# interactiveaudiolab/emphases

Hardware: AMD Instinct MI355X
Metric: utterances/s (10 s @16 kHz) whole-node (higher is better)
Workload: dtype f32; 1 GPU; 64 synthetic 10 s 16 kHz utterances per GPU, conv config, random word alignments, ragged batch with per-utterance (B=1) semantics (BASELINE.json configs[1]); utterances_per_gpu=64, frames_per_gpu=64000, words_per_gpu=1882, conv_tile=64, launch=hipGraph replay, batches_in_flight=2, parallelism=utterance-sharded x1, exchange=none (one rank)

## Files before the change

### emphases_amd/csrc/conv_stack.hip

```cpp
#include <type_traits>

#include "common.h"

#ifndef STACK_STAMP
#define STACK_STAMP(slot)
#endif

namespace emph {

typedef float f32x4 __attribute__((ext_vector_type(4)));
typedef float f32x2 __attribute__((ext_vector_type(2)));

constexpr int kStackChannels = 80;
constexpr int kStackMTiles = 5;
constexpr int kStackSteps = kStackChannels / 4;
constexpr int kStackChunkSteps = 4;
constexpr int kStackChunks = kStackSteps / kStackChunkSteps;
constexpr int kStackStepFloats = 6 * kStackMTiles * 64;
constexpr int kStackChunkFloats = kStackChunkSteps * kStackStepFloats;
constexpr int kStackWidth = 256;
constexpr int kStackStride = 260;
constexpr int kStackThreads = 768;
constexpr int kStackMaxLayers = 3;
constexpr int kSpanFields = 8;

__host__ __device__ constexpr int stack_lds_floats() {
    return kStackChannels * kStackStride + 2 * kStackChunkFloats +
           kStackMaxLayers * kStackChannels;
}

template <bool WORD_SUMS>
__global__ __launch_bounds__(kStackThreads) void conv1d_stack_kernel(
    const float* __restrict__ x, int64_t ldx, float* __restrict__ y, int64_t ldy,
    const float* __restrict__ packs, const float* __restrict__ biases, int layers,
    int relu_mask, const int32_t* __restrict__ spans, const int32_t* __restrict__ slot_map) {
    extern __shared__ __align__(16) float lds[];
    float* act = lds;
    float* ring = act + kStackChannels * kStackStride;
    float* bias_lds = ring + 2 * kStackChunkFloats;
    const int lane = threadIdx.x & 63;
    const int wave = __builtin_amdgcn_readfirstlane(threadIdx.x >> 6);
    const bool loader = wave >= 8;

    const int4 span_a = reinterpret_cast<const int4*>(spans)[2 * blockIdx.x];
    const int4 span_b = reinterpret_cast<const int4*>(spans)[2 * blockIdx.x + 1];
    const int owned_first = span_a.y;
    const int64_t column = span_a.z;
    const int count = span_a.w;
    const int owned = span_b.x;
    const int c0 = span_b.y;

    constexpr int kPackFloats = kStackSteps * kStackStepFloats;
    const int total_chunks = layers * kStackChunks;
    auto request = [&](int g, int first, int n) {
        const int layer = g / kStackChunks;
        const float* source = packs + static_cast<int64_t>(layer) * kPackFloats +
                              (g - layer * kStackChunks) * kStackChunkFloats;
        float* target = ring + (g & 1) * kStackChunkFloats;
        constexpr int kQuads = kStackChunkFloats / 4;
        const int each = (kQuads / 64 + n - 1) / n;
        for (int k = 0; k < each; ++k) {
            const int from = min(((wave - first) + k * n) * 64, kQuads - 64);
            __builtin_amdgcn_global_load_lds(
                (const __attribute__((address_space(1))) void*)(source + 4 * (from + lane)),
                (__attribute__((address_space(3))) void*)(target + 4 * from), 16, 0, 0);
        }
    };
    STACK_STAMP(0);

    const int last_quad = (count - 1) & ~3;
    auto fetch = [&](int c, int q) {
        const int p = c0 + 4 * q;
#ifdef STACK_NO_ROWS
        return make_float4(float(p), 0.f, 0.f, 0.f);
#endif
        return *reinterpret_cast<const float4*>(
            x + static_cast<int64_t>(c) * ldx + column + min(p, last_quad));
    };
    auto masked = [&](int q, const float4& v) {
        const int p = c0 + 4 * q;
        return make_float4(p < count ? v.x : 0.f, p + 1 < count ? v.y : 0.f,
                           p + 2 < count ? v.z : 0.f, p + 3 < count ? v.w : 0.f);
    };
    auto deposit = [&](int c, int q, const float4& raw) {
        const float4 v = masked(q, raw);
        float* target = act + c * kStackStride + 4 * q;
        target[1] = v.x;
        *reinterpret_cast<f32x2*>(target + 2) = f32x2{v.y, v.z};
        target[4] = v.w;
    };
    constexpr int kEarlyRows = 16;
    if (loader) {
        constexpr int kStage = 16 * 64 / 256;
        static_assert(kStage == 4, "the s_waitcnt below count these loads");
        f32x4 rows[kStackChunks - 1][kStage];
        float side[kStackChunks - 1];
        const int mine = threadIdx.x - 512;
        const int q = mine & 63;
        const int p = c0 + 4 * q;
        const float* source = x + static_cast<int64_t>(mine >> 6) * ldx + column + min(p, last_quad);
        const uint32_t target = static_cast<uint32_t>(reinterpret_cast<uintptr_t>(
            (__attribute__((address_space(3))) float*)(act + (mine >> 6) * kStackStride + 4 * q)));
        const int side_kind = mine < 64 ? (mine & 3) : 3;
        const int side_p = side_kind == 0 ? c0 - 1 : c0 + kStackWidth + side_kind - 1;
        const bool side_real = side_kind < 3 && side_p >= 0 && side_p < count;
        const float* side_source = x + static_cast<int64_t>((mine >> 2) & 15) * ldx + column +
                                   (side_real ? side_p : 0);
        const uint32_t side_target = static_cast<uint32_t>(reinterpret_cast<uintptr_t>(
            (__attribute__((address_space(3))) float*)(
                act + ((mine >> 2) & 15) * kStackStride +
                (side_kind == 0 ? 0 : kStackWidth + side_kind))));
        auto ask = [&](int chunk) {
#pragma unroll
            for (int round = 0; round < kStage; ++round) {
                const float* address = source + static_cast<int64_t>(16 * chunk + 4 * round) * ldx;
                asm volatile("global_load_dwordx4 %0, %1, off"
                             : "=v"(rows[chunk - 1][round]) : "v"(address) : "memory");
            }
            const float* address = side_source + static_cast<int64_t>(16 * chunk) * ldx;
            asm volatile("global_load_dword %0, %1, off" : "=v"(side[chunk - 1]) : "v"(address) : "memory");
        };
        auto hand_over = [&](int chunk) {
#pragma unroll
            for (int round = 0; round < kStage; ++round) {
                const f32x4 raw = rows[chunk - 1][round];
                const float first = p < count ? raw[0] : 0.f;
                const f32x2 middle = {p + 1 < count ? raw[1] : 0.f, p + 2 < count ? raw[2] : 0.f};
                const float last = p + 3 < count ? raw[3] : 0.f;
                const uint32_t address = target + (16 * chunk + 4 * round) * (kStackStride * 4);
                asm volatile(
                    "ds_write_b32 %0, %1 offset:4\n\t"
                    "ds_write_b64 %0, %2 offset:8\n\t"
                    "ds_write_b32 %0, %3 offset:16"
                    :
                    : "v"(address), "v"(first), "v"(middle), "v"(last)
                    : "memory");
            }
            const float beside = side_real ? side[chunk - 1] : 0.f;
            const uint32_t address = side_target + 16 * chunk * (kStackStride * 4);
            asm volatile("ds_write_b32 %0, %1" : : "v"(address), "v"(beside) : "memory");
        };
#define EMPH_ROWS_HERE(COUNT, STAGE)                                                        \
    asm volatile("s_waitcnt vmcnt(" #COUNT ")"                                              \
                 : "+v"(rows[STAGE][0]), "+v"(rows[STAGE][1]), "+v"(rows[STAGE][2]),        \
                   "+v"(rows[STAGE][3]), "+v"(side[STAGE])::"memory")
        request(1, 8, 4);
        ask(1);
        __builtin_amdgcn_s_barrier();
        ask(2);
        EMPH_ROWS_HERE(5, 0);
        hand_over(1);
        asm volatile("s_waitcnt lgkmcnt(0)" ::: "memory");
        __builtin_amdgcn_s_barrier();
        request(2, 8, 4);
        ask(3);
        EMPH_ROWS_HERE(13, 1);
        hand_over(2);
        asm volatile("s_waitcnt vmcnt(5) lgkmcnt(0)" ::: "memory");
        __builtin_amdgcn_s_barrier();
        request(3, 8, 4);
        ask(4);
        EMPH_ROWS_HERE(13, 2);
        hand_over(3);
        asm volatile("s_waitcnt vmcnt(5) lgkmcnt(0)" ::: "memory");
        __builtin_amdgcn_s_barrier();
        request(4, 8, 4);
        EMPH_ROWS_HERE(8, 3);
        hand_over(4);
#undef EMPH_ROWS_HERE
        for (int g = 4; g < total_chunks; ++g) {
            asm volatile("s_waitcnt vmcnt(0) lgkmcnt(0)" ::: "memory");
            STACK_STAMP(2 + 8 * (g / kStackChunks) + g % kStackChunks);
            __syncthreads();
            if (g + 1 < total_chunks) request(g + 1, 8, 4);
            if ((g + 1) % kStackChunks == 0 && g + 1 < total_chunks) __syncthreads();
        }
        return;
    }
    request(0, 0, 8);
    {
        static_assert(kStackMaxLayers * kStackChannels <= 512, "one bias per thread");
        const bool has_bias = threadIdx.x < layers * kStackChannels;
        const float bias_value = has_bias ? biases[threadIdx.x] : 0.f;
        constexpr int kEarly = kEarlyRows * 64 / 512;
        float4 early[kEarly];
#pragma unroll
        for (int round = 0; round < kEarly; ++round) {
            const int index = threadIdx.x + 512 * round;
            early[round] = fetch(index >> 6, index & 63);
        }
        float side = 0.f;
        const int side_row = threadIdx.x >> 2, side_kind = threadIdx.x & 3;
        if (side_row < kEarlyRows) {
            const float* row = x + static_cast<int64_t>(side_row) * ldx + column;
            const int p = side_kind == 0 ? c0 - 1 : c0 + kStackWidth + side_kind - 1;
            if (side_kind < 3 && p >= 0 && p < count) side = row[p];
        }
#pragma unroll
        for (int round = 0; round < kEarly; ++round) {
            const int index = threadIdx.x + 512 * round;
            deposit(index >> 6, index & 63, early[round]);
        }
        if (side_row < kEarlyRows)
            act[side_row * kStackStride + (side_kind == 0 ? 0 : kStackWidth + side_kind)] = side;
        if (has_bias) bias_lds[threadIdx.x] = bias_value;
    }
    STACK_STAMP(1);

    const int kk = lane >> 4;
    const int col = lane & 15;
    const int tile = wave & 3;
    const int part = wave >> 2;
    constexpr int split = (kStackMTiles + 1) >> 1;
    const int m_begin = part ? split : 0;
    const float* lane_rows = act + kk * kStackStride + 64 * tile + 4 * col;
    const int p_quad = c0 + 64 * tile + 4 * col;

    auto run = [&](auto count_tag) {
        constexpr int COUNT = decltype(count_tag)::value;
        for (int layer = 0; layer < layers; ++layer) {
            f32x4 acc[6][COUNT];
#pragma unroll
            for (int j = 0; j < 6; ++j)
#pragma unroll
                for (int m = 0; m < COUNT; ++m) acc[j][m] = f32x4{0.f, 0.f, 0.f, 0.f};
            float a[6][COUNT], d[6], v[6];
            auto load_b = [&](int step) {
                const float* source = lane_rows + 4 * step * kStackStride;
                const f32x4 first = *reinterpret_cast<const f32x4*>(source);
                const f32x2 second = *reinterpret_cast<const f32x2*>(source + 4);
                d[0] = first[0], d[1] = first[1], d[2] = first[2], d[3] = first[3];
                d[4] = second[0], d[5] = second[1];
            };
            for (int chunk = 0; chunk < kStackChunks; ++chunk) {
                __syncthreads();
                STACK_STAMP(2 + 8 * layer + chunk);
                if (chunk == 0 || layer == 0) load_b(chunk * kStackChunkSteps);
                const float* weights =
                    ring + ((layer * kStackChunks + chunk) & 1) * kStackChunkFloats +
                    (m_begin << 6) + lane;
#pragma unroll
                for (int ks = 0; ks < kStackChunkSteps; ++ks) {
                    const int step = chunk * kStackChunkSteps + ks;
#pragma unroll
                    for (int j = 0; j < 6; ++j)
#pragma unroll
                        for (int m = 0; m < COUNT; ++m)
#ifdef STACK_FEWER_A_READS
                            a[j][m] = (j & 1) ? a[j - 1][m]
                                              : weights[(ks * 6 * kStackMTiles + j * kStackMTiles + m) << 6];
#else
                            a[j][m] = weights[(ks * 6 * kStackMTiles + j * kStackMTiles + m) << 6];
#endif
#ifdef STACK_NO_TRANSFORM
                    for (int j = 0; j < 6; ++j) v[j] = d[j];
#else
                    const float p = fmaf(-4.f, d[2], d[4]);
                    const float q = fmaf(-4.f, d[1], d[3]);
                    const float c = d[4] - d[2];
                    const float e = 2.f * (d[3] - d[1]);
                    v[0] = fmaf(4.f, d[0], fmaf(-5.f, d[2], d[4]));
                    v[1] = p + q;
                    v[2] = p - q;
                    v[3] = c + e;
                    v[4] = c - e;
                    v[5] = fmaf(4.f, d[1], fmaf(-5.f, d[3], d[5]));
#endif
                    if (step + 1 < kStackSteps) load_b(step + 1);
#pragma unroll
                    for (int j = 0; j < 6; ++j)
#pragma unroll
                        for (int m = 0; m < COUNT; ++m)
                            acc[j][m] = __builtin_amdgcn_mfma_f32_16x16x4f32(
                                a[j][m], v[j], acc[j][m], 0, 0, 0);
                }
            }
            const bool relu = (relu_mask >> layer) & 1;
            const bool last = layer == layers - 1;
            const float* bias_row = bias_lds + layer * kStackChannels;
            STACK_STAMP(2 + 8 * layer + 5);
            if (!last) {
                __syncthreads();
#pragma unroll
                for (int m = 0; m < COUNT; ++m) {
                    const int channel0 = 16 * (m_begin + m) + 4 * kk;
                    const f32x4 add = *reinterpret_cast<const f32x4*>(bias_row + channel0);
#pragma unroll
                    for (int r = 0; r < 4; ++r) {
                        const float m1 = acc[1][m][r], m2 = acc[2][m][r];
                        const float m3 = acc[3][m][r], m4 = acc[4][m][r];
                        const float s12 = m1 + m2, d12 = m1 - m2, s34 = m3 + m4, d34 = m3 - m4;
                        float o0 = acc[0][m][r] + s12 + s34 + add[r];
                        float o1 = fmaf(2.f, d34, d12) + add[r];
                        float o2 = fmaf(4.f, s34, s12) + add[r];
                        float o3 = fmaf(8.f, d34, d12) + acc[5][m][r] + add[r];
                        if (relu) {
                            o0 = o0 < 0.f ? 0.f : o0;
                            o1 = o1 < 0.f ? 0.f : o1;
                            o2 = o2 < 0.f ? 0.f : o2;
                            o3 = o3 < 0.f ? 0.f : o3;
                        }
                        o0 = p_quad < count ? o0 : 0.f;
                        o1 = p_quad + 1 < count ? o1 : 0.f;
                        o2 = p_quad + 2 < count ? o2 : 0.f;
                        o3 = p_quad + 3 < count ? o3 : 0.f;
                        float* target =
                            act + (channel0 + r) * kStackStride + 64 * tile + 4 * col + 1;
                        target[0] = o0;
                        *reinterpret_cast<f32x2*>(target + 1) = f32x2{o1, o2};
                        target[3] = o3;
                    }
                }
                STACK_STAMP(2 + 8 * layer + 6);
                continue;
            }
            const int t = p_quad;
            const int owned_end = owned_first + owned;
            if (WORD_SUMS) {
                int4 slots = {-1, -1, -1, -1};
                if (t < count) slots = *reinterpret_cast<const int4*>(slot_map + column + t);
#pragma unroll
                for (int m = 0; m < COUNT; ++m) {
                    const int channel0 = 16 * (m_begin + m) + 4 * kk;
                    const f32x4 add = *reinterpret_cast<const f32x4*>(bias_row + channel0);
                    f32x4 sum[4];
#pragma unroll
                    for (int r = 0; r < 4; ++r) {
                        const float m1 = acc[1][m][r], m2 = acc[2][m][r];
                        const float m3 = acc[3][m][r], m4 = acc[4][m][r];
                        const float s12 = m1 + m2, d12 = m1 - m2, s34 = m3 + m4, d34 = m3 - m4;
                        float o0 = acc[0][m][r] + s12 + s34 + add[r];
                        float o1 = fmaf(2.f, d34, d12) + add[r];
                        float o2 = fmaf(4.f, s34, s12) + add[r];
                        float o3 = fmaf(8.f, d34, d12) + acc[5][m][r] + add[r];
                        if (relu) {
                            o0 = o0 < 0.f ? 0.f : o0;
                            o1 = o1 < 0.f ? 0.f : o1;
                            o2 = o2 < 0.f ? 0.f : o2;
                            o3 = o3 < 0.f ? 0.f : o3;
                        }
                        o0 = (t >= owned_first && t < owned_end) ? o0 : 0.f;
                        o1 = (t + 1 >= owned_first && t + 1 < owned_end) ? o1 : 0.f;
                        o2 = (t + 2 >= owned_first && t + 2 < owned_end) ? o2 : 0.f;
                        o3 = (t + 3 >= owned_first && t + 3 < owned_end) ? o3 : 0.f;
                        o1 += o0;
                        o2 += o1;
                        o3 += o2;
                        float scan = o3;
                        scan += __builtin_bit_cast(float, __builtin_amdgcn_update_dpp(
                            0, __builtin_bit_cast(int, scan), 0x111, 0xf, 0xf, true));
                        scan += __builtin_bit_cast(float, __builtin_amdgcn_update_dpp(
                            0, __builtin_bit_cast(int, scan), 0x112, 0xf, 0xf, true));
                        scan += __builtin_bit_cast(float, __builtin_amdgcn_update_dpp(
                            0, __builtin_bit_cast(int, scan), 0x114, 0xf, 0xf, true));
                        scan += __builtin_bit_cast(float, __builtin_amdgcn_update_dpp(
                            0, __builtin_bit_cast(int, scan), 0x118, 0xf, 0xf, true));
                        const float before = scan - o3;
                        sum[0][r] = o0 + before;
                        sum[1][r] = o1 + before;
                        sum[2][r] = o2 + before;
                        sum[3][r] = o3 + before;
                    }
#pragma unroll
                    for (int j = 0; j < 4; ++j) {
                        const int slot = j == 0 ? slots.x : j == 1 ? slots.y : j == 2 ? slots.z : slots.w;
                        if (slot >= 0 && t + j >= owned_first && t + j < owned_end)
                            *reinterpret_cast<f32x4*>(y + static_cast<int64_t>(slot) * ldy +
                                                      channel0) = sum[j];
                    }
                }
                continue;
            }
            const bool vector_ok = (ldy & 3) == 0 && (column & 3) == 0 &&
                                   (reinterpret_cast<uintptr_t>(y) & 15) == 0;
#pragma unroll
            for (int m = 0; m < COUNT; ++m) {
                const int channel0 = 16 * (m_begin + m) + 4 * kk;
                const f32x4 add = *reinterpret_cast<const f32x4*>(bias_row + channel0);
#pragma unroll
                for (int r = 0; r < 4; ++r) {
                    const float m1 = acc[1][m][r], m2 = acc[2][m][r];
                    const float m3 = acc[3][m][r], m4 = acc[4][m][r];
                    const float s12 = m1 + m2, d12 = m1 - m2, s34 = m3 + m4, d34 = m3 - m4;
                    float4 out;
                    out.x = acc[0][m][r] + s12 + s34 + add[r];
                    out.y = fmaf(2.f, d34, d12) + add[r];
                    out.z = fmaf(4.f, s34, s12) + add[r];
                    out.w = fmaf(8.f, d34, d12) + acc[5][m][r] + add[r];
                    if (relu) {
                        out.x = out.x < 0.f ? 0.f : out.x;
                        out.y = out.y < 0.f ? 0.f : out.y;
                        out.z = out.z < 0.f ? 0.f : out.z;
                        out.w = out.w < 0.f ? 0.f : out.w;
                    }
                    float* target = y + static_cast<int64_t>(channel0 + r) * ldy + column + t;
                    if (vector_ok && t >= owned_first && t + 3 < owned_end) {
                        *reinterpret_cast<float4*>(target) = out;
                    } else {
                        if (t >= owned_first && t < owned_end) target[0] = out.x;
                        if (t + 1 >= owned_first && t + 1 < owned_end) target[1] = out.y;
                        if (t + 2 >= owned_first && t + 2 < owned_end) target[2] = out.z;
                        if (t + 3 >= owned_first && t + 3 < owned_end) target[3] = out.w;
                    }
                }
            }
            STACK_STAMP(2 + 8 * layer + 6);
        }
    };
    if (part == 0) run(std::integral_constant<int, split>{});
    else run(std::integral_constant<int, kStackMTiles - split>{});
}

}

using namespace emph;

extern "C" {

int32_t emph_conv_stack_max_layers(void) { return kStackMaxLayers; }

int32_t emph_conv_stack_spans(const int64_t* host_counts, const int64_t* host_offsets,
                              int32_t n_segments, int32_t* host_spans) {
    int32_t total = 0;
    for (int32_t segment = 0; segment < n_segments; ++segment) {
        const int64_t count = host_counts[segment];
        if (count <= 0) continue;
        const int64_t quads = (count + 3) / 4;
        int64_t pieces = 1;
        if (quads > 64) {
            pieces = 2;
            while (2 * 63 + (pieces - 2) * 62 < quads) ++pieces;
        }
        const int64_t base = quads / pieces;
        int64_t spare = quads - base * pieces;
        int64_t extra[3] = {0, 0, 0};
        if (pieces > 1) {
            if (spare > 0 && base + 1 <= 63) extra[0] = 1, --spare;
            if (spare > 0 && base + 1 <= 63) extra[1] = 1, --spare;
            extra[2] = spare;
        }
        int64_t done = 0;
        for (int64_t k = 0; k < pieces; ++k) {
            int64_t share = base;
            if (pieces == 1) share = quads;
            else if (k == 0) share += extra[0];
            else if (k == pieces - 1) share += extra[1];
            else if (k <= extra[2]) share += 1;
            if (k == pieces - 1) share = quads - done;
            if (host_spans != nullptr) {
                int32_t* row = host_spans + static_cast<int64_t>(total) * kSpanFields;
                const int64_t first = 4 * done;
                int64_t owned = 4 * share;
                if (first + owned > count) owned = count - first;
                row[0] = segment;
                row[1] = static_cast<int32_t>(first);
                row[2] = static_cast<int32_t>(host_offsets[segment]);
                row[3] = static_cast<int32_t>(count);
                row[4] = static_cast<int32_t>(owned);
                row[5] = static_cast<int32_t>(first > 0 ? first - 4 : 0);
                row[6] = row[7] = 0;
            }
            done += share;
            ++total;
        }
    }
    return total;
}

int emph_conv1d_stack(const float* x, int64_t ldx, float* y, int64_t ldy, const float* packs,
                      const float* biases, int32_t layers, int32_t relu_mask,
                      const int32_t* spans, int32_t n_spans, const int32_t* slot_map,
                      void* stream) {
    if (n_spans == 0) return EMPH_OK;
    EMPH_REQUIRE(x && y && packs && biases && spans, EMPH_EINVAL,
                 "emph_conv1d_stack: null pointer");
    EMPH_REQUIRE(layers >= 1 && layers <= kStackMaxLayers, EMPH_ERANGE,
                 "emph_conv1d_stack: %d layers (1 .. %d)", layers, kStackMaxLayers);
    EMPH_REQUIRE((reinterpret_cast<uintptr_t>(x) & 15) == 0 && (ldx & 3) == 0, EMPH_EINVAL,
                 "emph_conv1d_stack: the input must be 16-byte aligned with ldx a multiple of 4");
    EMPH_REQUIRE(slot_map == nullptr ||
                     ((reinterpret_cast<uintptr_t>(y) & 15) == 0 && (ldy & 3) == 0 &&
                      ldy >= kStackChannels && (reinterpret_cast<uintptr_t>(slot_map) & 15) == 0),
                 EMPH_EINVAL, "emph_conv1d_stack: bad sums buffer or slot map");
    const size_t lds = static_cast<size_t>(stack_lds_floats()) * sizeof(float);
    hipStream_t s = static_cast<hipStream_t>(stream);
    if (slot_map != nullptr) {
        auto kernel = conv1d_stack_kernel<true>;
        static LdsReservation reserved;
        if (int status = reserve_lds(reserved, reinterpret_cast<const void*>(kernel), lds,
                                     "emph_conv1d_stack"))
            return status;
        EMPH_LAUNCH(kernel, dim3(n_spans), dim3(kStackThreads), lds, s, x, ldx, y, ldy, packs,
                    biases, layers, relu_mask, spans, slot_map);
    } else {
        auto kernel = conv1d_stack_kernel<false>;
        static LdsReservation reserved;
        if (int status = reserve_lds(reserved, reinterpret_cast<const void*>(kernel), lds,
                                     "emph_conv1d_stack"))
            return status;
        EMPH_LAUNCH(kernel, dim3(n_spans), dim3(kStackThreads), lds, s, x, ldx, y, ldy, packs,
                    biases, layers, relu_mask, spans, slot_map);
    }
    return check_launch("emph_conv1d_stack");
}

}
```

### emphases_amd/csrc/forward.hip

```cpp
#include "common.h"

using namespace emph;

namespace emph {
__global__ __launch_bounds__(64) void launch_probe_kernel() {}
}

extern "C" {

int emph_launch_probe(void* stream) {
    EMPH_LAUNCH(launch_probe_kernel, dim3(1), dim3(64), 0, static_cast<hipStream_t>(stream));
    return check_launch("emph_launch_probe");
}

int64_t emph_prominence_workspace_floats(int32_t features, int32_t channels,
                                         int64_t ld_frames, int64_t ld_words,
                                         int32_t n_slots) {
    return (static_cast<int64_t>(features) + 2 * channels) * ld_frames +
           static_cast<int64_t>(channels) * (ld_words + n_slots);
}

int emph_prominence_forward(const emph_conv_model* model, const void* audio,
                            int32_t audio_format, const int64_t* seg,
                            const int32_t* frontend_tiles,
                            int32_t n_frontend_tiles, const int32_t* frame_tiles,
                            int32_t n_frame_tiles, int32_t tile_n,
                            const int32_t* word_tiles, int32_t n_word_tiles,
                            const int32_t* bounds, const int32_t* word_segment,
                            int64_t ld_frames, int64_t ld_words, float* workspace,
                            float* logits, float* scores,
                            const emph_word_sum_tables* word_sums,
                            const int32_t* conv_spans, int32_t n_conv_spans, void* stream) {
    EMPH_REQUIRE(model != nullptr, EMPH_EINVAL, "emph_prominence_forward: model is null");
    const emph_conv_model& m = *model;
    EMPH_REQUIRE(audio && seg && workspace, EMPH_EINVAL,
                 "emph_prominence_forward: null pointer");
    EMPH_REQUIRE(m.features == kMels, EMPH_ERANGE,
                 "emph_prominence_forward: %d feature rows (the fused path takes the 80 mel "
                 "rows only)", m.features);
    EMPH_REQUIRE(m.encoder_layers >= 0 && m.encoder_layers <= 16, EMPH_ERANGE,
                 "emph_prominence_forward: %d encoder layers", m.encoder_layers);
    const bool quad = m.conv_variant == 1;
    EMPH_REQUIRE(m.conv_variant == 0 || quad, EMPH_EINVAL,
                 "emph_prominence_forward: conv_variant %d", m.conv_variant);
    EMPH_REQUIRE(!quad || tile_n == 64, EMPH_ERANGE,
                 "emph_prominence_forward: F(4,3) takes 64-position tiles, not %d", tile_n);
    const int64_t lds_square = quad ? emph_conv_winograd4_lds_bytes(m.channels, m.channels)
                                    : emph_conv_winograd_lds_bytes(m.channels, m.channels);
    const int64_t lds_input = quad ? emph_conv_winograd4_lds_bytes(m.channels, m.features)
                                   : emph_conv_winograd_lds_bytes(m.channels, m.features);
    EMPH_REQUIRE(lds_square <= 160 * 1024 && lds_input <= 160 * 1024, EMPH_ERANGE,
                 "emph_prominence_forward: %d channels do not fit the Winograd kernel's LDS",
                 m.channels);
    const int c = m.channels;
    float* features = workspace;
    float* current = features + static_cast<int64_t>(m.features) * ld_frames;
    float* other = current + static_cast<int64_t>(c) * ld_frames;
    float* words = other + static_cast<int64_t>(c) * ld_frames;
    float* sums = words + static_cast<int64_t>(c) * ld_words;
    const bool fold = word_sums != nullptr && m.encoder_layers > 0;
    EMPH_REQUIRE(!fold || (quad && (m.reduction == EMPH_REDUCE_SUM ||
                                    m.reduction == EMPH_REDUCE_AVERAGE)),
                 EMPH_EINVAL,
                 "emph_prominence_forward: word_sums needs conv_variant 1 and a sum / average "
                 "reduction");

    int status = emph_logmel(audio, audio_format, seg, frontend_tiles, n_frontend_tiles, m.table,
                             m.mel_start, m.mel_count, m.mel_offset, m.mel_values, m.mel_nnz,
                             features, ld_frames, 0, -1, nullptr, nullptr, m.normalize, stream);
    if (status) return status;
    auto conv = [&](const float* in, float* out, const float* pack, const float* bias, int c_in,
                    int activation) {
        return quad ? emph_conv1d_winograd4(in, ld_frames, out, ld_frames, pack, bias, c_in, c,
                                            activation, frame_tiles, n_frame_tiles, stream)
                    : emph_conv1d_winograd(in, ld_frames, out, ld_frames, pack, bias, c_in, c,
                                           activation, frame_tiles, n_frame_tiles, tile_n,
                                           stream);
    };
    const int64_t pack_floats =
        quad ? emph_conv_winograd4_pack_size(c, c) : emph_conv_winograd_pack_size(c, c);
    const bool stack = conv_spans != nullptr && quad && c == 80 && m.features == 80 &&
                       m.encoder_packs == m.input_pack + pack_floats &&
                       m.encoder_biases == m.input_bias + c &&
                       (m.activation == EMPH_ACT_RELU || m.activation == EMPH_ACT_NONE);
    if (stack) {
        const int total = 1 + m.encoder_layers;
        const int most = emph_conv_stack_max_layers();
        const int groups = (total + most - 1) / most;
        float* buffers[2] = {current, other};
        const float* in = features;
        int done = 0;
        for (int group = 0; group < groups; ++group) {
            const int size = (total - done + (groups - group) - 1) / (groups - group);
            int relu = 0;
            for (int l = 0; l < size; ++l)
                if (done + l >= 1 && m.activation == EMPH_ACT_RELU) relu |= 1 << l;
            const bool to_sums = group == groups - 1 && fold;
            float* out = to_sums ? sums : buffers[group & 1];
            status = emph_conv1d_stack(in, ld_frames, out, to_sums ? c : ld_frames,
                                       m.input_pack + done * pack_floats,
                                       m.input_bias + static_cast<int64_t>(done) * c, size, relu,
                                       conv_spans, n_conv_spans,
                                       to_sums ? word_sums->slot_map : nullptr, stream);
            if (status) return status;
            in = out;
            done += size;
        }
        current = const_cast<float*>(in);
        status = fold ? emph_word_sums(sums, c, word_sums->terms, word_sums->first,
                                       word_sums->lengths, words, ld_words, c, ld_words,
                                       m.reduction, stream)
                      : emph_segment_reduce(current, ld_frames, bounds, words, ld_words, c, seg,
                                            word_segment, ld_words, m.reduction, stream);
        if (status) return status;
        return emph_word_decoder(words, ld_words, word_tiles, n_word_tiles, c, m.decoder_packs,
                                 m.decoder_biases, m.decoder_layers, m.decoder_kernel_size,
                                 m.activation, m.out_weight, m.out_bias, m.decoder_kernel_size,
                                 m.post, logits, scores, stream);
    }
    status = conv(features, current, m.input_pack, m.input_bias, m.features, EMPH_ACT_NONE);
    if (status) return status;
    for (int layer = 0; layer < m.encoder_layers; ++layer) {
        if (fold && layer == m.encoder_layers - 1) {
            status = emph_conv1d_winograd4_word_sums(
                current, ld_frames, sums, c, m.encoder_packs + layer * pack_floats,
                m.encoder_biases + static_cast<int64_t>(layer) * c, c, c, m.activation,
                frame_tiles, n_frame_tiles, word_sums->slot_map, stream);
            if (status) return status;
            break;
        }
        status = conv(current, other, m.encoder_packs + layer * pack_floats,
                      m.encoder_biases + static_cast<int64_t>(layer) * c, c, m.activation);
        if (status) return status;
        float* swap = current;
        current = other;
        other = swap;
    }
    status = fold ? emph_word_sums(sums, c, word_sums->terms, word_sums->first,
                                   word_sums->lengths, words, ld_words, c, ld_words,
                                   m.reduction, stream)
                  : emph_segment_reduce(current, ld_frames, bounds, words, ld_words, c, seg,
                                        word_segment, ld_words, m.reduction, stream);
    if (status) return status;
    return emph_word_decoder(words, ld_words, word_tiles, n_word_tiles, c, m.decoder_packs,
                             m.decoder_biases, m.decoder_layers, m.decoder_kernel_size,
                             m.activation, m.out_weight, m.out_bias, m.decoder_kernel_size,
                             m.post, logits, scores, stream);
}

}
```

### emphases_amd/engine.py

```python
import contextlib
import functools
import os
import ctypes
import threading

import numpy as np
import torch

from . import config as cfg
from . import melbasis
from . import runtime
from . import weights as weights_module

FRONTEND_BLOCK = None
PRECISIONS = {'f32': (0, 0, 0), 'bf16x3': (2, 32, 3), 'bf16x3_fast': (2, 32, 2),
              'bf16x6': (0, 3, 3)}
ATTENTION_BLOCK = 64
ATTENTION_GROUP = 256
GROUPED_FROM = ATTENTION_GROUP // 2
FUSED_WORDS = 64
EVERYTHING = 1 << 30
SHORT, LONG = (0, GROUPED_FROM - 1), (GROUPED_FROM, EVERYTHING)
FEW_WORDS, MANY_WORDS = (0, FUSED_WORDS), (FUSED_WORDS + 1, EVERYTHING)
WORD_TILE = 16
WINOGRAD_LDS_BUDGET = 160 * 1024
SPLIT16_COLUMNS = 1 << 22
KERNEL_COLUMNS = 1 << 28
HEAD_DIMS = (32, 40, 64)


TRACKS_NEEDED = (
    'pitch/periodicity features come from the third-party '
    '`penn` tracker; pass its outputs as tracks '
    '[2, ld_frames] (see core.from_alignments_and_audios '
    'pitch_tracker=)')


def check_supported(config):
    channels = config.channels
    if channels > 128:
        raise ValueError(f'channels {channels} > 128: the word reduce and '
                         'the LayerNorm hold at most 128 channels')
    if config.architecture == 'transformer':
        head_dim = channels // config.heads
        if head_dim not in HEAD_DIMS:
            raise ValueError(
                f'head dimension {head_dim} (channels {channels} / heads '
                f'{config.heads}) not in {{32, 40, 64}}')
    elif config.layers > 16:
        raise ValueError(f'{config.layers} convolution layers > 16')
    if config.architecture == 'convolution' or not config.has_decoder:
        if channels < 16 or channels % 16:
            raise ValueError(
                f'channels {channels} not a multiple of 16 in 16..128 (the '
                'fused word stage of this configuration)')
        if config.decoder_kernel_size not in (1, 3, 5):
            raise ValueError(
                f'decoder kernel size {config.decoder_kernel_size} not in '
                '{1, 3, 5} (the fused word stage of this configuration)')
        layers = config.layers if config.has_decoder else 0
        if runtime.library().emph_word_decoder_block(
                layers, config.decoder_kernel_size,
                config.decoder_kernel_size) < 16:
            raise ValueError(
                f'{layers} decoder layers of kernel size '
                f'{config.decoder_kernel_size}: the receptive field is too '
                "wide for the fused word stage's 64-word window")


def a_weighting():
    frequencies = np.fft.rfftfreq(n=1024, d=1.0 / 8000)
    f_sq = frequencies ** 2.0
    const = np.array([12194.217, 20.598997, 107.65265, 737.86223]) ** 2.0
    with np.errstate(divide='ignore'):
        weights = 2.0 + 20.0 * (
            np.log10(const[0]) + 2 * np.log10(f_sq)
            - np.log10(f_sq + const[0]) - np.log10(f_sq + const[1])
            - 0.5 * np.log10(f_sq + const[2])
            - 0.5 * np.log10(f_sq + const[3]))
    return (np.maximum(-80.0, weights) - cfg.REF_DB).astype(np.float32)


class _Conv:

    def __init__(self, weight, bias, device, winograd=False):
        weight = np.asarray(weight, dtype=np.float32)
        if weight.ndim == 2:
            weight = weight[:, :, None]
        self.c_out, self.c_in, self.kernel_size = weight.shape
        self.weight = weight
        self.pack = torch.from_numpy(runtime.conv_pack(weight)).to(device)
        self.winograd = None
        if winograd and self.kernel_size == 3 and \
                runtime.conv_winograd_lds_bytes(self.c_out, self.c_in) <= \
                WINOGRAD_LDS_BUDGET:
            self.winograd = torch.from_numpy(
                runtime.conv_winograd_pack(weight)).to(device)
        self.winograd4 = None
        if winograd and self.kernel_size == 3 and self.c_out <= 96 and \
                self.c_in % 4 == 0 and \
                runtime.conv_winograd4_lds_bytes(self.c_out, self.c_in) <= \
                WINOGRAD_LDS_BUDGET:
            self.winograd4 = torch.from_numpy(
                runtime.conv_winograd4_pack(weight)).to(device)
        self.bias = None if bias is None else torch.from_numpy(
            np.ascontiguousarray(bias, dtype=np.float32)).to(device)


class Engine:

    def __init__(self, config=cfg.DEFAULT, state=None, device=None,
                 conv_tile=None, winograd=True, precision='f32'):
        if precision not in PRECISIONS:
            raise ValueError(
                f'precision {precision!r} is not one of {sorted(PRECISIONS)}')
        check_supported(config)
        self.config = config
        self.precision = precision
        self.split_pieces, self.attention_pieces, self.linear_pieces = \
            PRECISIONS[precision]
        self.winograd = winograd
        self.device = runtime.require_gpu(device)
        self.lib = runtime.library()
        global FRONTEND_BLOCK
        FRONTEND_BLOCK = int(self.lib.emph_frontend_block())
        self.conv_tile = conv_tile
        self.timers = None
        self._workspace = {}
        self._staging = {}
        self.lock = threading.RLock()
        self.split_tile = int(os.environ.get('EMPHASES_SPLIT_TILE', 16))
        if self.split_tile not in (16, 32):
            raise ValueError('EMPHASES_SPLIT_TILE must be 16 or 32')
        self.max_columns = SPLIT16_COLUMNS if (
            config.architecture == 'transformer' and self.linear_pieces and
            self.split_tile == 16) else KERNEL_COLUMNS
        state = weights_module.load(state, config)
        self.state = state
        dev = self.device
        to = lambda a: torch.from_numpy(np.ascontiguousarray(a)).to(dev)

        self.table = to(runtime.frontend_table())
        basis = melbasis.default()
        self.mel_start = to(basis.row_start)
        self.mel_count = to(basis.row_count)
        self.mel_offset = to(basis.row_offset)
        self.mel_values = to(basis.values)
        self.mel_nnz = int(basis.values.size)
        self.a_weights = to(a_weighting())

        self.input_layer = _Conv(
            state['input_layer.weight'], state['input_layer.bias'], dev,
            winograd)
        self.frame_encoder = self._stack('frame_encoder')
        self.word_decoder = self._stack('word_decoder') \
            if config.has_decoder else None
        self.output_weight = to(state['output_layer.weight'])
        self.output_bias = to(state['output_layer.bias'])
        self.fused_words = config.architecture == 'convolution' or \
            not config.has_decoder
        self.word_block = WORD_TILE
        if self.fused_words:
            layers = self.word_decoder if config.has_decoder else []
            self.decoder_layers = len(layers)
            self.decoder_packs = torch.from_numpy(np.concatenate([
                runtime.word_decoder_pack(l.weight) for l in layers])).to(dev) \
                if layers else None
            self.decoder_biases = torch.cat([l.bias for l in layers]) \
                if layers else None
            self.word_block = int(self.lib.emph_word_decoder_block(
                self.decoder_layers, config.decoder_kernel_size,
                config.decoder_kernel_size))
            self.decoder_tiles = (runtime.AXIS_DECODER, (
                self.decoder_layers, config.decoder_kernel_size,
                config.decoder_kernel_size))
        if config.architecture == 'transformer':
            self.position = to(weights_module.positional_encoding(
                cfg.MAX_POSITIONS, config.channels))
            self.position_rows = self.position.t().contiguous()
        self.word_transformer = None
        if config.architecture == 'transformer' and config.has_decoder and \
                config.channels in (64, 80) and config.heads == 2 and all(
                    tuple(state[f'word_decoder.model.layers.{i}.{name}.weight']
                          .shape) == (config.channels, config.channels)
                    for i in range(config.layers)
                    for name in ('linear1', 'linear2')):
            self.word_transformer = to(np.concatenate([
                runtime.word_transformer_pack(
                    state, f'word_decoder.model.layers.{i}.', config.channels,
                    config.heads) for i in range(config.layers)]))
        frame_layers = [self.input_layer] + (
            self.frame_encoder if config.architecture == 'convolution' else [])
        self.fuse_qkv = os.environ.get('EMPHASES_FUSE_QKV', '1') != '0'
        self.quad = winograd and config.activation in (None, 'relu') and \
            all(layer.winograd4 is not None for layer in frame_layers)
        self.fold = bool(
            self.quad and config.architecture == 'convolution' and
            config.downsample_location != 'input' and
            config.downsample_method in ('sum', 'average') and
            len(self.frame_encoder) > 0 and config.channels % 4 == 0 and
            os.environ.get('EMPHASES_FOLD_WORD_SUMS', '1') != '0')
        frame_stack = [self.input_layer] + list(self.frame_encoder) \
            if config.architecture == 'convolution' else []
        self.stack = bool(
            self.quad and frame_stack and
            config.downsample_location != 'input' and
            all(layer.c_in == 80 and layer.c_out == 80 and
                layer.kernel_size == 3 and layer.winograd4 is not None
                for layer in frame_stack) and
            os.environ.get('EMPHASES_CONV_STACK', '1') != '0')
        if self.stack:
            self._stack_packs = torch.cat(
                [layer.winograd4 for layer in frame_stack])
            self._stack_biases = torch.cat(
                [layer.bias for layer in frame_stack])
        self.split_conv = bool(self.stack and self.split_pieces == 2)
        self.sum_step = 32 if self.split_conv else 64
        if self.split_conv:
            self._split_packs = to(np.concatenate(
                [runtime.conv_split_pack(layer.weight) for layer in frame_stack]))
        self.model = self._conv_model()

    def lane(self):
        import copy
        other = copy.copy(self)
        other._workspace = {}
        other._staging = {}
        other.timers = None
        other.lock = threading.RLock()
        return other

    def _conv_model(self):
        config = self.config
        layers = [self.input_layer] + (
            self.frame_encoder if config.architecture == 'convolution' else [])
        if config.architecture != 'convolution' or not self.winograd or \
                config.downsample_location == 'input' or \
                config.num_features != cfg.NUM_MELS or \
                any(layer.winograd is None for layer in layers):
            return None
        encoder = self.frame_encoder
        pick = (lambda l: l.winograd4) if self.quad else (lambda l: l.winograd)
        input_pack, input_bias = pick(self.input_layer), self.input_layer.bias
        if self.stack:
            size = input_pack.numel()
            input_pack = self._stack_packs[:size]
            self._encoder_packs = self._stack_packs[size:]
            input_bias = self._stack_biases[:config.channels]
            self._encoder_biases = self._stack_biases[config.channels:]
        else:
            self._encoder_packs = torch.cat([pick(l) for l in encoder]) \
                if encoder else torch.zeros(1, device=self.device)
            self._encoder_biases = torch.cat([l.bias for l in encoder]) \
                if encoder else torch.zeros(1, device=self.device)
        pointer = lambda t: None if t is None else t.data_ptr()
        return runtime.ConvModel(
            channels=config.channels, features=config.num_features,
            encoder_layers=len(encoder), decoder_layers=self.decoder_layers,
            decoder_kernel_size=config.decoder_kernel_size,
            activation=runtime.ACTIVATIONS[config.activation],
            reduction=runtime.REDUCTIONS[config.downsample_method],
            post=runtime.POSTPROCESS[config.loss],
            normalize=int(config.normalize), mel_nnz=self.mel_nnz,
            conv_variant=int(self.quad),
            table=pointer(self.table), mel_start=pointer(self.mel_start),
            mel_count=pointer(self.mel_count),
            mel_offset=pointer(self.mel_offset),
            mel_values=pointer(self.mel_values),
            input_pack=pointer(input_pack),
            input_bias=pointer(input_bias),
            encoder_packs=pointer(self._encoder_packs),
            encoder_biases=pointer(self._encoder_biases),
            decoder_packs=pointer(self.decoder_packs),
            decoder_biases=pointer(self.decoder_biases),
            out_weight=pointer(self.output_weight),
            out_bias=pointer(self.output_bias))

    def _stack(self, prefix):
        config, state, dev = self.config, self.state, self.device
        layers = []
        if config.architecture == 'convolution':
            for i in range(config.layers):
                layers.append(_Conv(
                    state[f'{prefix}.{2 * i}.weight'],
                    state[f'{prefix}.{2 * i}.bias'], dev,
                    self.winograd and prefix == 'frame_encoder'))
            return layers
        channels = config.channels
        to = lambda a: torch.from_numpy(np.ascontiguousarray(a)).to(dev)
        for i in range(config.layers):
            p = f'{prefix}.model.layers.{i}.'
            in_w = state[p + 'self_attn.in_proj_weight']
            in_b = state[p + 'self_attn.in_proj_bias']
            block = None
            square = (channels, channels)
            if channels in (64, 80) and all(
                    tuple(state[p + name].shape) == square for name in (
                        'self_attn.out_proj.weight', 'linear1.weight',
                        'linear2.weight')):
                block = (
                    to(np.concatenate([
                        runtime.linear_chain_pack(
                            state[p + 'self_attn.out_proj.weight'], True),
                        runtime.linear_chain_pack(
                            state[p + 'linear1.weight'], False),
                        runtime.linear_chain_pack(
                            state[p + 'linear2.weight'], False)])),
                    to(np.concatenate([
                        state[p + name].astype(np.float32) for name in (
                            'self_attn.out_proj.bias', 'norm1.weight',
                            'norm1.bias', 'linear1.bias', 'linear2.bias',
                            'norm2.weight', 'norm2.bias')])))
            qkv = None
            if channels in (64, 80):
                qkv = (to(np.concatenate([
                    runtime.linear_chain_pack(
                        in_w[part * channels:(part + 1) * channels], True)
                    for part in range(3)])), to(in_b.astype(np.float32)))
            block_split = qkv_split = None
            if self.linear_pieces and channels == 80 and config.heads == 2 and \
                    block is not None:
                pieces = self.linear_pieces
                pack = functools.partial(
                    runtime.linear_split_pack, pieces=pieces,
                    tile=self.split_tile)
                block_split = (
                    to(np.concatenate([
                        pack(state[p + name])
                        for name in ('self_attn.out_proj.weight',
                                     'linear1.weight', 'linear2.weight')])),
                    block[1])
                qkv_split = (to(np.concatenate([
                    pack(in_w[part * channels:(part + 1) * channels])
                    for part in range(3)])), qkv[1])
            layers.append(dict(
                block=block, qkv=qkv, block_split=block_split,
                qkv_split=qkv_split,
                qk=_Conv(in_w[:2 * channels], in_b[:2 * channels], dev),
                v=_Conv(in_w[2 * channels:], in_b[2 * channels:], dev),
                out=_Conv(state[p + 'self_attn.out_proj.weight'],
                          state[p + 'self_attn.out_proj.bias'], dev),
                linear1=_Conv(state[p + 'linear1.weight'],
                              state[p + 'linear1.bias'], dev),
                linear2=_Conv(state[p + 'linear2.weight'],
                              state[p + 'linear2.bias'], dev),
                norm1=(to(state[p + 'norm1.weight']),
                       to(state[p + 'norm1.bias'])),
                norm2=(to(state[p + 'norm2.weight']),
                       to(state[p + 'norm2.bias']))))
        for i in range(config.layers - 1):
            p = f'{prefix}.model.layers.{i + 1}.'
            block = layers[i]['block']
            layers[i]['block_qkv'] = None
            if block is None or layers[i + 1]['qkv'] is None or \
                    (6 * channels * channels + 10 * channels) * 4 > 160 * 1024:
                continue
            in_w = state[p + 'self_attn.in_proj_weight']
            in_b = state[p + 'self_attn.in_proj_bias']
            layers[i]['block_qkv'] = (
                torch.cat([block[0]] + [to(runtime.linear_chain_pack(
                    in_w[part * channels:(part + 1) * channels], False))
                    for part in range(3)]),
                torch.cat([block[1], to(in_b.astype(np.float32))]))
        if layers:
            layers[-1]['block_qkv'] = None
        return layers


    def frame_tile(self, plan):
        if self.conv_tile is not None and self.conv_tile != 'auto':
            return self.conv_tile
        if self.conv_tile is None and self.quad:
            return 64
        frames = [segment.frames for segment in plan.segments]
        if self.winograd:
            cost = {64: 20.7 if self.quad else 26.7, 32: 23.2, 16: 16.1}
        else:
            cost = {64: 33.5, 32: 31.3, 16: 16.1}
        candidates = (64, 32, 16) if self.quad else (32, 64, 16)
        if self.conv_tile is None and self.winograd:
            candidates = (32, 64)
        best = None
        for tile in candidates:
            tiles = sum(-(-count // tile) for count in frames)
            waves = 4 if tile == 64 else 8
            if tile == 64 and self.quad:
                waves = 4
            groups = -(-tiles // waves)
            trips = -(-groups // 256)
            if best is None or trips * cost[tile] < best[0]:
                best = (trips * cost[tile], tile)
        return best[1]

    def _pinned(self, name, array):
        slots = self._staging.setdefault(name, [[], 0])
        ring, cursor = slots
        if len(ring) < 4:
            ring.append(None)
        index = cursor % len(ring)
        slots[1] = cursor + 1
        tensor = ring[index]
        if tensor is None or tensor.numel() < array.size:
            tensor = torch.empty(
                max(array.size, 1) * 3 // 2, dtype=torch.int32).pin_memory()
            ring[index] = tensor
        view = tensor[:array.size]
        np.copyto(view.numpy(), array)
        return view

    def prepare(self, plan):
        if self.config.downsample_location != 'input':
            tile = self.frame_tile(plan)
            plan.prepared = (tile,) + self._pack(plan, tile, False)
        return plan

    def _pack(self, plan, tile, nested):
        requests = [
            (runtime.AXIS_FRAMES, FRONTEND_BLOCK),
            (runtime.AXIS_FRAMES, tile),
            self.decoder_tiles if self.fused_words
            else (runtime.AXIS_WORDS, self.word_block)]
        if self.config.architecture == 'transformer':
            requests += [(runtime.AXIS_FRAMES, ATTENTION_BLOCK),
                         (runtime.AXIS_FRAMES, ATTENTION_BLOCK) + SHORT,
                         (runtime.AXIS_FRAMES, ATTENTION_GROUP) + LONG,
                         (runtime.AXIS_FRAMES, 32)]
            if self.linear_pieces:
                requests += [(runtime.AXIS_FRAMES, self.split_tile)]
            if not nested:
                requests += [(runtime.AXIS_WORDS, ATTENTION_BLOCK)]
                if self.word_transformer is not None:
                    requests += [
                        (runtime.AXIS_WORDS, ATTENTION_BLOCK) + FEW_WORDS,
                        (runtime.AXIS_WORDS, ATTENTION_BLOCK) + MANY_WORDS,
                        (runtime.AXIS_WORDS, self.word_block) + MANY_WORDS]
        requests = list(dict.fromkeys(requests))
        fold = self.fold and not nested and tile == 64
        stack = self.stack and not nested and tile == 64
        host, offsets = plan.pack_metadata(
            requests, word_sums=fold, spans=stack, sum_step=self.sum_step)
        return host, offsets, fold, stack

    def upload(self, plan, tile=None, nested=False):
        tile = tile or self.frame_tile(plan)
        prepared = getattr(plan, 'prepared', None)
        if prepared is not None and prepared[0] == tile and not nested:
            host, offsets, fold, stack = prepared[1:]
        else:
            host, offsets, fold, stack = self._pack(plan, tile, nested)
        pinned = self._pinned(('meta', nested), host)
        device_buffer = pinned.to(self.device, non_blocking=True)
        views = {'_buffer': device_buffer, '_pinned': pinned, 'tile': tile,
                 'positions': (plan.total_frames, plan.total_words)}
        for name, (start, size) in offsets.items():
            views[name] = (device_buffer[start:start + size], size)
        if fold:
            views['n_slots'] = plan.word_sum_tables(
                plan.stack_restarts(self.sum_step)
                if stack else None)['n_slots']
            views['word_sum_tables'] = runtime.WordSumTables(
                *[views[('word_sums', name)][0].data_ptr() for name in (
                    'slot_map', 'terms', 'first', 'lengths')],
                views['n_slots'])
        if self.config.downsample_location == 'input' and not nested and \
                len(plan):
            pieces = plan.pieces(self.config.downsample_method)
            piece_meta = self.upload(
                pieces.plan, self.frame_tile(pieces.plan), nested=True)
            extra = self._pinned('pieces', np.concatenate([
                pieces.gather.view(np.int32).ravel(),
                pieces.bounds.ravel(), pieces.word_piece,
                pieces.gather[:, 1].astype(np.int32)]))
            extra = extra.to(self.device, non_blocking=True)
            cut = pieces.gather.size * 2
            piece_meta['gather'] = extra[:cut]
            piece_meta['piece_bounds'] = extra[cut:cut + pieces.bounds.size]
            cut += pieces.bounds.size
            piece_meta['word_piece'] = extra[cut:cut + pieces.word_piece.size]
            piece_meta['key_counts'] = extra[cut + pieces.word_piece.size:]
            piece_meta['plan'] = pieces.plan
            piece_meta['_extra'] = extra
            views['pieces'] = piece_meta
        return views


    @contextlib.contextmanager
    def _timed(self, name, flops=0.):
        if self.timers is None:
            yield
            return
        begin = torch.cuda.Event(enable_timing=True)
        end = torch.cuda.Event(enable_timing=True)
        first = self.lib.emph_launch_timer_count()
        begin.record()
        yield
        end.record()
        self.timers.append((name, flops, begin, end, first,
                            self.lib.emph_launch_timer_count()))

    def _buffer(self, name, *shape):
        key = (name, shape)
        tensor = self._workspace.get(key)
        if tensor is None:
            for stale in [k for k in self._workspace if k[0] == name]:
                del self._workspace[stale]
            tensor = torch.empty(shape, dtype=torch.float32, device=self.device)
            self._workspace[key] = tensor
        return tensor

    def pack_audio(self, audios):
        lengths = [int(audio.shape[0]) for audio in audios]
        total = sum(lengths)
        packed = self._buffer('packed_audio', max(total, 1))[:total]
        offset = 0
        for audio, length in zip(audios, lengths):
            packed[offset:offset + length].copy_(audio, non_blocking=True)
            offset += length
        return packed

    def _conv(self, layer, x, ldx, y, ldy, meta, axis, block, activation,
              transpose_out=False, position=False):
        tiles, size = meta[('tiles', axis, block)]
        positions = meta['positions'][axis]
        name = (f'conv1d_{"frames" if axis == runtime.AXIS_FRAMES else "words"}'
                f'_{layer.c_in}x{layer.c_out}_k{layer.kernel_size}')
        flops = 2. * layer.c_in * layer.c_out * layer.kernel_size * positions
        bias = None if layer.bias is None else layer.bias.data_ptr()
        if layer.winograd4 is not None and axis == runtime.AXIS_FRAMES and \
                block == 64 and self.quad and not transpose_out and \
                activation in (None, 'relu'):
            with self._timed(name.replace('conv1d', 'conv1d_winograd4'), flops):
                if position:
                    runtime.check(self.lib.emph_conv1d_winograd4_position(
                        x.data_ptr(), ldx, y.data_ptr(), ldy,
                        layer.winograd4.data_ptr(), bias, layer.c_in,
                        layer.c_out, runtime.ACTIVATIONS[activation],
                        tiles.data_ptr(), size // runtime.TILE_FIELDS,
                        self.position_rows.data_ptr(), cfg.MAX_POSITIONS,
                        runtime.stream()), 'emph_conv1d_winograd4_position')
                    return True
                runtime.check(self.lib.emph_conv1d_winograd4(
                    x.data_ptr(), ldx, y.data_ptr(), ldy,
                    layer.winograd4.data_ptr(), bias, layer.c_in, layer.c_out,
                    runtime.ACTIVATIONS[activation], tiles.data_ptr(),
                    size // runtime.TILE_FIELDS, runtime.stream()),
                    'emph_conv1d_winograd4')
            return False
        if layer.winograd is not None and axis == runtime.AXIS_FRAMES and \
                block in (32, 64) and not transpose_out:
            with self._timed(name.replace('conv1d', 'conv1d_winograd'), flops):
                runtime.check(self.lib.emph_conv1d_winograd(
                    x.data_ptr(), ldx, y.data_ptr(), ldy,
                    layer.winograd.data_ptr(), bias, layer.c_in, layer.c_out,
                    runtime.ACTIVATIONS[activation], tiles.data_ptr(),
                    size // runtime.TILE_FIELDS, block, runtime.stream()),
                    'emph_conv1d_winograd')
            return False
        with self._timed(name, flops):
            runtime.check(self.lib.emph_conv1d(
                x.data_ptr(), ldx, y.data_ptr(), ldy, layer.pack.data_ptr(),
                bias, layer.c_in, layer.c_out, layer.kernel_size,
                runtime.ACTIVATIONS[activation], tiles.data_ptr(),
                size // runtime.TILE_FIELDS, block, int(transpose_out),
                runtime.stream()), 'emph_conv1d')
        return False

    def features(self, audio, plan, meta, tracks=None, config=None, out=None):
        config = config or self.config
        rows = config.num_features
        if out is None:
            out = self._buffer('features', rows, plan.ld_frames)
        elif out.shape[0] < rows or out.stride(0) != plan.ld_frames or \
                out.dtype != torch.float32:
            raise ValueError('features: out must be float32 rows of ld_frames')
        mel_row = 0 if config.mel_feature else -1
        loud_row = rows - 1 if config.loudness_feature else -1
        if config.pitch_feature or config.periodicity_feature:
            if tracks is None or tuple(tracks.shape) != (2, plan.ld_frames):
                raise NotImplementedError(TRACKS_NEEDED)
            first = cfg.NUM_MELS if config.mel_feature else 0
            pitch_row = first if config.pitch_feature else -1
            periodicity_row = first + int(config.pitch_feature) \
                if config.periodicity_feature else -1
            with self._timed('pitch_rows'):
                runtime.check(self.lib.emph_pitch_rows(
                    tracks[0].data_ptr(), tracks[1].data_ptr(),
                    out.data_ptr(), plan.ld_frames, pitch_row,
                    periodicity_row, int(config.normalize),
                    float(np.log2(np.float32(cfg.FMIN))),
                    float(np.log2(np.float32(cfg.FMAX))), runtime.stream()),
                    'emph_pitch_rows')
        tiles, size = meta[('tiles', runtime.AXIS_FRAMES, FRONTEND_BLOCK)]
        count = size // runtime.TILE_FIELDS
        table = meta['table'][0]
        peak = None
        if config.loudness_feature:
            peak = torch.zeros(
                len(plan), dtype=torch.float32, device=self.device)
            with self._timed('frontend_peak'):
                runtime.check(self.lib.emph_frontend_peak(
                    audio.data_ptr(), audio_format(audio), table.data_ptr(),
                    tiles.data_ptr(),
                    count, self.table.data_ptr(), peak.data_ptr(),
                    runtime.stream()), 'emph_frontend_peak')
        if mel_row >= 0 or loud_row >= 0:
            with self._timed('frontend_logmel'):
                runtime.check(self.lib.emph_logmel(
                    audio.data_ptr(), audio_format(audio), table.data_ptr(),
                    tiles.data_ptr(),
                    count, self.table.data_ptr(), self.mel_start.data_ptr(),
                    self.mel_count.data_ptr(), self.mel_offset.data_ptr(),
                    self.mel_values.data_ptr(), self.mel_nnz, out.data_ptr(),
                    plan.ld_frames, mel_row, loud_row,
                    None if peak is None else peak.data_ptr(),
                    self.a_weights.data_ptr(), int(config.normalize),
                    runtime.stream()), 'emph_logmel')
        return out

    def _transformer(self, layers, x, ld, plan, meta, axis, block, tag,
                     key_counts=None, positioned=False, select=()):
        config = self.config
        channels = config.channels
        if block > 32 and ('tiles', axis, 32) + select in meta:
            block = 32
        att_tiles, att_size = meta[('tiles', axis, ATTENTION_BLOCK) + select]
        att_count = att_size // runtime.TILE_FIELDS
        if att_count == 0:
            return x
        counts = plan.frames if axis == runtime.AXIS_FRAMES else plan.words
        if len(counts) and int(counts.max()) > cfg.MAX_POSITIONS:
            raise RuntimeError(
                f'a chunk of {int(counts.max())} positions exceeds the '
                f'{cfg.MAX_POSITIONS}-entry positional encoding; pass a '
                'smaller batch_size')
        if not positioned:
            with self._timed('add_position'):
                runtime.check(self.lib.emph_add_position(
                    x.data_ptr(), ld, self.position.data_ptr(), channels,
                    cfg.MAX_POSITIONS, att_tiles.data_ptr(), att_count,
                    ATTENTION_BLOCK, runtime.stream()), 'emph_add_position')
        qk = self._buffer(tag + '_qk', 2 * channels, ld)
        v = self._buffer(tag + '_v', ld, channels)
        attended = self._buffer(tag + '_attended', channels, ld)
        projected = self._buffer(tag + '_projected', channels, ld)
        attention_flops = 4. * channels * float(
            (counts.astype(np.float64) ** 2).sum())
        launches = [(att_tiles, att_count, ATTENTION_BLOCK)]
        if axis == runtime.AXIS_FRAMES and not select and \
                ('tiles', axis, ATTENTION_GROUP) + LONG in meta:
            launches = []
            for key, size in (((ATTENTION_BLOCK,) + SHORT, ATTENTION_BLOCK),
                              ((ATTENTION_GROUP,) + LONG, ATTENTION_GROUP)):
                tiles, length = meta[('tiles', axis) + key]
                if length:
                    launches.append(
                        (tiles, length // runtime.TILE_FIELDS, size))

        def add_layernorm(norm):
            with self._timed('add_layernorm'):
                runtime.check(self.lib.emph_add_layernorm(
                    x.data_ptr(), projected.data_ptr(), x.data_ptr(), ld,
                    channels, norm[0].data_ptr(), norm[1].data_ptr(),
                    config.layer_norm_eps, 0, ld, runtime.stream()),
                    'emph_add_layernorm')

        split_images = None
        if self.attention_pieces and config.channels // config.heads == 40 and \
                any(tile_n == ATTENTION_GROUP for _, _, tile_n in launches):
            size = int(self.lib.emph_split_kv_bytes(
                ld, len(plan), channels, config.heads,
                self.attention_pieces))
            key = (tag + '_split_kv', (size,))
            split_images = self._workspace.get(key)
            if split_images is None:
                for stale in [k for k in self._workspace if k[0] == key[0]]:
                    del self._workspace[stale]
                split_images = torch.empty(
                    size, dtype=torch.uint8, device=self.device)
                self._workspace[key] = split_images

        projected_images = split_images is not None and \
            all(tile_n == ATTENTION_GROUP for _, _, tile_n in launches)

        def attend(images_written):
            for tiles, count, tile_n in launches:
                counts_pointer = None if key_counts is None else \
                    key_counts.data_ptr()
                if split_images is not None and tile_n == ATTENTION_GROUP:
                    if not images_written:
                        runtime.check(self.lib.emph_split_kv(
                            qk.data_ptr(), v.data_ptr(), ld, channels,
                            config.heads, att_tiles.data_ptr(), att_count,
                            ATTENTION_BLOCK, self.attention_pieces,
                            split_images.data_ptr(), runtime.stream()),
                            'emph_split_kv')
                    runtime.check(self.lib.emph_attention_split(
                        qk.data_ptr(), split_images.data_ptr(),
                        attended.data_ptr(), ld, channels, config.heads,
                        tiles.data_ptr(), count, tile_n, counts_pointer,
                        self.attention_pieces, runtime.stream()),
                        'emph_attention_split')
                    continue
                runtime.check(self.lib.emph_attention(
                    qk.data_ptr(), v.data_ptr(), attended.data_ptr(), ld,
                    channels, config.heads, tiles.data_ptr(), count, tile_n,
                    counts_pointer, runtime.stream()), 'emph_attention')

        split_tiles, wide = None, self.split_tile
        if axis == runtime.AXIS_FRAMES and ('tiles', axis, wide) + select in meta:
            split_tiles = meta[('tiles', axis, wide) + select]

        def position_wise(layer, following):
            tiles, size = split_tiles
            block_packs, vectors = layer['block_split'] if layer else (None, None)
            next_packs, next_bias = following['qkv_split'] if following \
                else (None, None)
            pointer = lambda t: None if t is None else t.data_ptr()
            runtime.check(self.lib.emph_position_wise_split(
                attended.data_ptr() if layer else None, x.data_ptr(), ld,
                channels, config.heads, pointer(block_packs), pointer(vectors),
                pointer(next_packs), pointer(next_bias), self.linear_pieces,
                self.attention_pieces, config.layer_norm_eps,
                runtime.ACTIVATIONS['relu'], tiles.data_ptr(),
                size // runtime.TILE_FIELDS, 16, qk.data_ptr(), v.data_ptr(),
                split_images.data_ptr() if projected_images and following
                else None, runtime.stream()), 'emph_position_wise_split')

        projected_ahead = False
        images_ahead = False
        for index, layer in enumerate(layers):
            split = layer['block_split'] is not None and \
                split_tiles is not None and block <= 32
            images_written = False
            if projected_ahead:
                images_written = images_ahead
            elif split:
                packs, bias = layer['qkv_split']
                tiles, size = split_tiles
                with self._timed(f'qkv_projection_split_{tag}', 6. * channels *
                                 channels * meta['positions'][axis]):
                    if wide == 16:
                        position_wise(None, layer)
                        images_written = projected_images
                    elif projected_images:
                        runtime.check(self.lib.emph_qkv_projection_split_images(
                            x.data_ptr(), ld, qk.data_ptr(),
                            split_images.data_ptr(), channels, config.heads,
                            packs.data_ptr(), self.linear_pieces,
                            self.attention_pieces, bias.data_ptr(),
                            tiles.data_ptr(), size // runtime.TILE_FIELDS, 32,
                            runtime.stream()),
                            'emph_qkv_projection_split_images')
                        images_written = True
                    else:
                        runtime.check(self.lib.emph_qkv_projection_split(
                            x.data_ptr(), ld, qk.data_ptr(), v.data_ptr(),
                            channels, packs.data_ptr(), self.linear_pieces,
                            bias.data_ptr(), tiles.data_ptr(),
                            size // runtime.TILE_FIELDS, 32, runtime.stream()),
                            'emph_qkv_projection_split')
            elif layer['qkv'] is not None and block <= 32:
                packs, bias = layer['qkv']
                tiles, size = meta[('tiles', axis, block) + select]
                with self._timed(f'qkv_projection_{tag}', 6. * channels * channels *
                                 meta['positions'][axis]):
                    runtime.check(self.lib.emph_qkv_projection(
                        x.data_ptr(), ld, qk.data_ptr(), v.data_ptr(),
                        channels, packs.data_ptr(), bias.data_ptr(),
                        tiles.data_ptr(), size // runtime.TILE_FIELDS, block,
                        runtime.stream()), 'emph_qkv_projection')
            else:
                self._conv(layer['qk'], x, ld, qk, ld, meta, axis, block,
                           None)
                self._conv(layer['v'], x, ld, v, channels, meta, axis, block,
                           None, transpose_out=True)
            projected_ahead = False
            with self._timed(f'attention_{tag}', attention_flops):
                attend(images_written)
            following = layers[index + 1] if index + 1 < len(layers) else None
            if split and following is not None and self.fuse_qkv and \
                    following['block_split'] is not None:
                packs, vectors = layer['block_split']
                next_packs, next_bias = following['qkv_split']
                tiles, size = split_tiles
                with self._timed(f'transformer_block_qkv_split_{tag}', 12. *
                                 channels * channels * meta['positions'][axis]):
                    if wide == 16:
                        position_wise(layer, following)
                    else:
                        runtime.check(self.lib.emph_transformer_block_qkv_split(
                            attended.data_ptr(), x.data_ptr(), ld, channels,
                            config.heads, packs.data_ptr(), next_packs.data_ptr(),
                            self.linear_pieces, self.attention_pieces,
                            vectors.data_ptr(), next_bias.data_ptr(),
                            config.layer_norm_eps, runtime.ACTIVATIONS['relu'],
                            tiles.data_ptr(), size // runtime.TILE_FIELDS, 32,
                            qk.data_ptr(), v.data_ptr(),
                            split_images.data_ptr() if projected_images else None,
                            runtime.stream()), 'emph_transformer_block_qkv_split')
                projected_ahead, images_ahead = True, projected_images
                continue
            if split:
                packs, vectors = layer['block_split']
                tiles, size = split_tiles
                with self._timed(f'transformer_block_split_{tag}', 6. * channels *
                                 channels * meta['positions'][axis]):
                    if wide == 16:
                        position_wise(layer, None)
                    else:
                        runtime.check(self.lib.emph_transformer_block_split(
                            attended.data_ptr(), x.data_ptr(), ld, channels,
                            packs.data_ptr(), self.linear_pieces, vectors.data_ptr(),
                            config.layer_norm_eps, runtime.ACTIVATIONS['relu'],
                            tiles.data_ptr(), size // runtime.TILE_FIELDS, 32,
                            runtime.stream()), 'emph_transformer_block_split')
                continue
            if layer['block_qkv'] is not None and block <= 32 and self.fuse_qkv:
                packs, vectors = layer['block_qkv']
                tiles, size = meta[('tiles', axis, block) + select]
                with self._timed(f'transformer_block_qkv_{tag}', 12. * channels *
                                 channels * meta['positions'][axis]):
                    runtime.check(self.lib.emph_transformer_block_qkv(
                        attended.data_ptr(), x.data_ptr(), ld, channels,
                        packs.data_ptr(), vectors.data_ptr(),
                        config.layer_norm_eps, runtime.ACTIVATIONS['relu'],
                        tiles.data_ptr(), size // runtime.TILE_FIELDS, block,
                        qk.data_ptr(), v.data_ptr(), runtime.stream()),
                        'emph_transformer_block_qkv')
                projected_ahead = True
                continue
            if layer['block'] is not None and block <= 32:
                packs, vectors = layer['block']
                tiles, size = meta[('tiles', axis, block) + select]
                with self._timed(f'transformer_block_{tag}', 6. * channels *
                                 channels * meta['positions'][axis]):
                    runtime.check(self.lib.emph_transformer_block(
                        attended.data_ptr(), x.data_ptr(), ld, channels,
                        packs.data_ptr(), vectors.data_ptr(),
                        config.layer_norm_eps, runtime.ACTIVATIONS['relu'],
                        tiles.data_ptr(), size // runtime.TILE_FIELDS, block,
                        runtime.stream()), 'emph_transformer_block')
                continue
            self._conv(layer['out'], attended, ld, projected, ld, meta, axis,
                       block, None)
            add_layernorm(layer['norm1'])
            self._conv(layer['linear1'], x, ld, attended, ld, meta, axis,
                       block, 'relu')
            self._conv(layer['linear2'], attended, ld, projected, ld, meta,
                       axis, block, None)
            add_layernorm(layer['norm2'])
        return x

    def _frame_stack(self, features, ld_f, a, b, out, ld_w, plan, meta,
                     frames=True, words=True):
        config = self.config
        channels = config.channels
        spans, span_size = meta['conv_spans']
        total = 1 + len(self.frame_encoder)
        most = int(self.lib.emph_conv_stack_max_layers())
        groups = -(-total // most)
        fold = 'word_sum_tables' in meta
        view = lambda name: meta[('word_sums', name)][0]
        sums = self._buffer(
            'word_sums', max(meta.get('n_slots', 0), 1), channels)
        pack = self.input_layer.winograd4.numel()
        relu_layers = config.activation == 'relu'
        source, buffers, done = features, (a, b), 0
        if self.split_conv:
            groups = -(-total // 5)
            split_bytes = int(self.lib.emph_conv_split_pack_size())
        for group in range(groups if frames else 0):
            size = -(-(total - done) // (groups - group))
            relu = sum(1 << l for l in range(size)
                       if done + l >= 1 and relu_layers)
            to_sums = fold and group == groups - 1
            target = sums if to_sums else buffers[group & 1]
            flops = 2. * 80 * 80 * 3 * plan.total_frames * size
            if self.split_conv:
                with self._timed('conv1d_split_frames_80x80_k3', flops):
                    runtime.check(self.lib.emph_conv1d_split(
                        source.data_ptr(), ld_f, target.data_ptr(),
                        channels if to_sums else ld_f,
                        self._split_packs[done * split_bytes:].data_ptr(),
                        self._stack_biases[done * channels:].data_ptr(), size,
                        relu, spans.data_ptr(), span_size // 8,
                        view('slot_map').data_ptr() if to_sums else None,
                        runtime.stream()), 'emph_conv1d_split')
                source = target
                done += size
                continue
            with self._timed('conv1d_stack_frames_80x80_k3', flops):
                runtime.check(self.lib.emph_conv1d_stack(
                    source.data_ptr(), ld_f, target.data_ptr(),
                    channels if to_sums else ld_f,
                    self._stack_packs[done * pack:].data_ptr(),
                    self._stack_biases[done * channels:].data_ptr(), size,
                    relu, spans.data_ptr(), span_size // 8,
                    view('slot_map').data_ptr() if to_sums else None,
                    runtime.stream()), 'emph_conv1d_stack')
            source = target
            done += size
        if not words:
            return
        if fold:
            with self._timed('word_sums'):
                runtime.check(self.lib.emph_word_sums(
                    sums.data_ptr(), channels, view('terms').data_ptr(),
                    view('first').data_ptr(), view('lengths').data_ptr(),
                    out.data_ptr(), ld_w, channels, ld_w,
                    runtime.REDUCTIONS[config.downsample_method],
                    runtime.stream()), 'emph_word_sums')
        else:
            with self._timed('segment_reduce'):
                runtime.check(self.lib.emph_segment_reduce(
                    source.data_ptr(), ld_f, meta['bounds'][0].data_ptr(),
                    out.data_ptr(), ld_w, channels,
                    meta['table'][0].data_ptr(),
                    meta['word_segment'][0].data_ptr(), ld_w,
                    runtime.REDUCTIONS[config.downsample_method],
                    runtime.stream()), 'emph_segment_reduce')

    def _word_sums(self, x, ld_f, out, ld_w, plan, meta):
        config = self.config
        layer = self.frame_encoder[-1]
        channels = config.channels
        tiles, size = meta[('tiles', runtime.AXIS_FRAMES, 64)]
        sums = self._buffer('word_sums', max(meta['n_slots'], 1), channels)
        view = lambda name: meta[('word_sums', name)][0]
        flops = 2. * layer.c_in * layer.c_out * 3 * plan.total_frames
        with self._timed(
                f'conv1d_winograd4_frames_{layer.c_in}x{layer.c_out}_k3', flops):
            runtime.check(self.lib.emph_conv1d_winograd4_word_sums(
                x.data_ptr(), ld_f, sums.data_ptr(), channels,
                layer.winograd4.data_ptr(), layer.bias.data_ptr(), layer.c_in,
                layer.c_out, runtime.ACTIVATIONS[config.activation],
                tiles.data_ptr(), size // runtime.TILE_FIELDS,
                view('slot_map').data_ptr(), runtime.stream()),
                'emph_conv1d_winograd4_word_sums')
        with self._timed('word_sums'):
            runtime.check(self.lib.emph_word_sums(
                sums.data_ptr(), channels, view('terms').data_ptr(),
                view('first').data_ptr(), view('lengths').data_ptr(),
                out.data_ptr(), ld_w, channels, ld_w,
                runtime.REDUCTIONS[config.downsample_method],
                runtime.stream()), 'emph_word_sums')

    def _stack_forward(self, layers, x, other, ld, plan, meta, axis, block,
                       tag, key_counts=None, positioned=False):
        config = self.config
        if config.architecture == 'convolution':
            for layer in layers:
                self._conv(layer, x, ld, other, ld, meta, axis, block,
                           config.activation)
                x, other = other, x
            return x
        if axis == runtime.AXIS_WORDS and self.word_transformer is not None \
                and key_counts is None and len(plan.words):
            tiles, size = meta[('tiles', axis, ATTENTION_BLOCK) + FEW_WORDS]
            if size:
                with self._timed('word_transformer'):
                    runtime.check(self.lib.emph_word_transformer(
                        x.data_ptr(), ld, self.position.data_ptr(),
                        cfg.MAX_POSITIONS, config.channels, config.heads,
                        self.word_transformer.data_ptr(), len(layers),
                        config.layer_norm_eps, tiles.data_ptr(),
                        size // runtime.TILE_FIELDS, runtime.stream()),
                        'emph_word_transformer')
            if int(plan.words.max()) > FUSED_WORDS:
                self._transformer(
                    layers, x, ld, plan, meta, axis, block, tag, key_counts,
                    positioned, select=MANY_WORDS)
            return x
        return self._transformer(
            layers, x, ld, plan, meta, axis, block, tag, key_counts, positioned)


    def forward(self, audio, plan, meta=None, stages=None, features=None,
                tracks=None):
        config = self.config
        runs = self.sub_plans(plan)
        if runs is not None:
            if stages is not None:
                raise ValueError(
                    'stages of a plan past the packed-axis limit: pass its '
                    'segments in smaller plans')
            return self._forward_runs(audio, plan, runs, tracks, features)
        meta = meta or self.upload(plan)
        block = meta['tile']
        channels = config.channels
        ld_f, ld_w = plan.ld_frames, plan.ld_words
        frames, words = runtime.AXIS_FRAMES, runtime.AXIS_WORDS
        if self.model is not None and stages is None and features is None \
                and self.timers is None and not self.split_conv and \
                block in ((64,) if self.quad else (32, 64)) and \
                len(plan):
            check_bounds(plan, config.downsample_method)
            logits = self._buffer('logits', ld_w)
            scores = self._buffer('scores', ld_w)
            tables = meta.get('word_sum_tables')
            spans, span_size = meta.get('conv_spans', (None, 0))
            floats = self.lib.emph_prominence_workspace_floats(
                config.num_features, channels, ld_f, ld_w,
                meta.get('n_slots', 0))
            workspace = self._buffer('fused', int(floats))
            frontend_tiles, frontend_size = meta[
                ('tiles', frames, FRONTEND_BLOCK)]
            frame_tiles, frame_size = meta[('tiles', frames, block)]
            word_tiles, word_size = meta[('tiles',) + self.decoder_tiles]
            runtime.check(self.lib.emph_prominence_forward(
                ctypes.byref(self.model), audio.data_ptr(),
                audio_format(audio), meta['table'][0].data_ptr(),
                frontend_tiles.data_ptr(),
                frontend_size // runtime.TILE_FIELDS, frame_tiles.data_ptr(),
                frame_size // runtime.TILE_FIELDS, block,
                word_tiles.data_ptr(), word_size // runtime.TILE_FIELDS,
                meta['bounds'][0].data_ptr(),
                meta['word_segment'][0].data_ptr(), ld_f, ld_w,
                workspace.data_ptr(), logits.data_ptr(), scores.data_ptr(),
                None if tables is None else ctypes.byref(tables),
                spans.data_ptr() if spans is not None else None,
                span_size // 8 if spans is not None else 0,
                runtime.stream()), 'emph_prominence_forward')
            return scores, logits
        if features is None:
            features = self.features(audio, plan, meta, tracks=tracks)
        table = meta['table'][0]
        logits = self._buffer('logits', ld_w)
        scores = self._buffer('scores', ld_w)
        wa = self._buffer('words_a', channels, ld_w)
        if config.downsample_location == 'input':
            if stages is not None:
                stages['features'] = features.clone()
            piece_meta = meta['pieces']
            piece_plan = piece_meta['plan']
            ld_p = piece_plan.ld_frames
            gathered = self._buffer(
                'piece_features', config.num_features, ld_p)
            with self._timed('gather_columns'):
                runtime.check(self.lib.emph_gather_columns(
                    features.data_ptr(), ld_f, gathered.data_ptr(), ld_p,
                    config.num_features, piece_meta['gather'].data_ptr(),
                    len(piece_plan), runtime.stream()),
                    'emph_gather_columns')
            a = self._buffer('frames_a', channels, ld_p)
            b = self._buffer('frames_b', channels, ld_p)
            self._conv(self.input_layer, gathered, ld_p, a, ld_p, piece_meta,
                       frames, piece_meta['tile'], None)
            encoded = self._stack_forward(
                self.frame_encoder, a, b, ld_p, piece_plan, piece_meta,
                frames, piece_meta['tile'], 'pieces',
                key_counts=piece_meta['key_counts']
                if config.architecture == 'transformer' else None)
            with self._timed('segment_reduce'):
                runtime.check(self.lib.emph_segment_reduce(
                    encoded.data_ptr(), ld_p,
                    piece_meta['piece_bounds'].data_ptr(), wa.data_ptr(),
                    ld_w, channels, piece_meta['table'][0].data_ptr(),
                    piece_meta['word_piece'].data_ptr(), ld_w,
                    runtime.REDUCTIONS[config.downsample_method],
                    runtime.stream()), 'emph_segment_reduce')
        else:
            a = self._buffer('frames_a', channels, ld_f)
            b = self._buffer('frames_b', channels, ld_f)
            if 'conv_spans' in meta and stages is None:
                check_bounds(plan, config.downsample_method)
                self._frame_stack(features, ld_f, a, b, wa, ld_w, plan, meta)
            else:
                positioned = self._conv(
                    self.input_layer, features, ld_f, a, ld_f, meta, frames, block,
                    None, position=config.architecture == 'transformer' and
                    stages is None)
                if stages is not None:
                    stages['features'] = features.clone()
                    stages['input_layer'] = a.clone()
                fold = 'word_sum_tables' in meta and stages is None
                encoded = self._stack_forward(
                    self.frame_encoder[:-1] if fold else self.frame_encoder, a, b,
                    ld_f, plan, meta, frames, block, 'frames',
                    positioned=positioned)
                if stages is not None:
                    stages['encoder'] = encoded.clone()

                check_bounds(plan, config.downsample_method)
                if fold:
                    self._word_sums(encoded, ld_f, wa, ld_w, plan, meta)
                else:
                    with self._timed('segment_reduce'):
                        runtime.check(self.lib.emph_segment_reduce(
                            encoded.data_ptr(), ld_f,
                            meta['bounds'][0].data_ptr(), wa.data_ptr(), ld_w,
                            channels, table.data_ptr(),
                            meta['word_segment'][0].data_ptr(), ld_w,
                            runtime.REDUCTIONS[config.downsample_method],
                            runtime.stream()), 'emph_segment_reduce')
        if stages is not None:
            stages['downsampled'] = wa.clone()
        return self._word_stage(wa, plan, meta, logits, scores)

    def sub_plans(self, plan):
        from . import batch
        pieces = self.config.downsample_location == 'input' and len(plan)
        if plan.ld_frames < self.max_columns and (not pieces or plan.pieces(
                self.config.downsample_method).plan.ld_frames <
                self.max_columns):
            return None
        room = self.max_columns - batch.LEAD - batch.TAIL
        columns = [-(-plan.frames // batch.ALIGN) * batch.ALIGN]
        if pieces:
            first = np.cumsum(plan.words) - plan.words
            longest = np.array([
                int(np.max(plan.segment_bounds[1, f:f + n] -
                           plan.segment_bounds[0, f:f + n])) if n else 0
                for f, n in zip(first, plan.words)], dtype=np.int64)
            columns.append(plan.words * (
                -(-longest // batch.ALIGN) * batch.ALIGN))
        columns = np.stack(columns)
        if (columns >= room).any():
            raise ValueError(
                f'one segment fills {int(columns.max())} packed columns, '
                f'more than the {room} of a pass')
        runs, first, used = [], 0, np.zeros(len(columns), dtype=np.int64)
        for index in range(len(plan)):
            if (used + columns[:, index] >= room).any():
                runs.append((first, index))
                first, used = index, 0 * used
            used += columns[:, index]
        runs.append((first, len(plan)))
        return runs

    def _forward_runs(self, audio, plan, runs, tracks, features=None):
        from . import batch
        table = plan.table
        scores = self._buffer('whole_scores', plan.ld_words)
        logits = self._buffer('whole_logits', plan.ld_words)
        first_word = np.cumsum(plan.words) - plan.words
        for first, end in runs:
            rows = slice(first, end)
            count = end - first
            words = plan.words[rows]
            bounds = plan.segment_bounds[
                :, first_word[first]:first_word[first] + int(words.sum())]
            part = batch.Plan.from_columns(
                np.arange(count, dtype=np.int64), plan.start_word[rows],
                table[rows, runtime.SEG_START], table[rows, runtime.SEG_LENGTH],
                plan.frames[rows], words, bounds,
                table[rows, runtime.SEG_AUDIO_OFF],
                table[rows, runtime.SEG_AUDIO_LEN])

            def repack(rows):
                if rows is None:
                    return None
                out = torch.zeros((rows.shape[0], part.ld_frames),
                                  dtype=rows.dtype, device=rows.device)
                for i in range(count):
                    at, n = int(plan.frame_off[first + i]), int(part.frames[i])
                    to = int(part.frame_off[i])
                    out[:, to:to + n] = rows[:, at:at + n]
                return out
            part_scores, part_logits = self.forward(
                audio, part, tracks=repack(tracks), features=repack(features))
            at, size = int(plan.word_off[first]), part.ld_words - batch.LEAD - \
                batch.TAIL
            scores[at:at + size].copy_(
                part_scores[batch.LEAD:batch.LEAD + size])
            logits[at:at + size].copy_(
                part_logits[batch.LEAD:batch.LEAD + size])
        return scores, logits

    def _word_stage(self, wa, plan, meta, logits, scores):
        config = self.config
        channels = config.channels
        ld_w = plan.ld_words
        words = runtime.AXIS_WORDS
        table = meta['table'][0]
        if self.fused_words:
            tiles, size = meta[('tiles',) + self.decoder_tiles]
            with self._timed('word_decoder', 2. * channels * (
                    channels * config.decoder_kernel_size * self.decoder_layers
                    + config.decoder_kernel_size) * plan.total_words):
                runtime.check(self.lib.emph_word_decoder(
                    wa.data_ptr(), ld_w, tiles.data_ptr(),
                    size // runtime.TILE_FIELDS, channels,
                    None if self.decoder_packs is None
                    else self.decoder_packs.data_ptr(),
                    None if self.decoder_biases is None
                    else self.decoder_biases.data_ptr(),
                    self.decoder_layers, config.decoder_kernel_size,
                    runtime.ACTIVATIONS[config.activation],
                    self.output_weight.data_ptr(), self.output_bias.data_ptr(),
                    config.decoder_kernel_size,
                    runtime.POSTPROCESS[config.loss], logits.data_ptr(),
                    scores.data_ptr(), runtime.stream()), 'emph_word_decoder')
            return scores, logits
        wb = self._buffer('words_b', channels, ld_w)
        decoded = self._stack_forward(
            self.word_decoder, wa, wb, ld_w, plan, meta, words,
            self.word_block, 'words')
        with self._timed('output_layer'):
            runtime.check(self.lib.emph_output_layer(
                decoded.data_ptr(), ld_w, self.output_weight.data_ptr(),
                self.output_bias.data_ptr(), channels,
                config.decoder_kernel_size, table.data_ptr(),
                meta['word_segment'][0].data_ptr(), ld_w, words,
                runtime.POSTPROCESS[config.loss], logits.data_ptr(),
                scores.data_ptr(), runtime.stream()), 'emph_output_layer')
        return scores, logits

    def splittable(self, plan, meta):
        return (self.config.downsample_location != 'input' and
                'conv_spans' in meta and 'word_sum_tables' in meta and
                self.fused_words and len(plan) > 0 and
                self.sub_plans(plan) is None)

    def forward_frames(self, audio, plan, meta):
        ld_f = plan.ld_frames
        channels = self.config.channels
        check_bounds(plan, self.config.downsample_method)
        features = self.features(audio, plan, meta)
        a = self._buffer('frames_a', channels, ld_f)
        b = self._buffer('frames_b', channels, ld_f)
        self._frame_stack(features, ld_f, a, b, None, plan.ld_words, plan, meta,
                          words=False)

    def forward_words(self, plan, meta):
        ld_w = plan.ld_words
        logits = self._buffer('logits', ld_w)
        scores = self._buffer('scores', ld_w)
        wa = self._buffer('words_a', self.config.channels, ld_w)
        self._frame_stack(None, plan.ld_frames, None, None, wa, ld_w, plan, meta,
                          frames=False)
        return self._word_stage(wa, plan, meta, logits, scores)

    def capture(self, audio, plan, meta=None):
        if self.sub_plans(plan) is not None:
            raise ValueError('a plan past the packed-axis limit runs as '
                             'sub-plans: it cannot be captured as one graph')
        meta = meta or self.upload(plan)
        self.timers = None
        side = torch.cuda.Stream(device=self.device)
        side.wait_stream(torch.cuda.current_stream())
        with torch.cuda.stream(side):
            for _ in range(2):
                self.forward(audio, plan, meta)
        torch.cuda.current_stream().wait_stream(side)
        graph = torch.cuda.CUDAGraph()
        with torch.cuda.graph(graph, capture_error_mode='thread_local'):
            scores, logits = self.forward(audio, plan, meta)
        held = (list(self._workspace.values()), meta, audio)

        def replay():
            graph.replay()
            return held[0] is not None
        return replay, scores, logits


def audio_format(audio):
    if audio.dtype == torch.float32:
        return runtime.AUDIO_F32
    if audio.dtype == torch.int16:
        return runtime.AUDIO_PCM16
    raise TypeError(f'packed audio must be float32 or int16, not {audio.dtype}')


def check_bounds(plan, method):
    if method not in ('max', 'center'):
        return
    for segment in plan.segments:
        starts, ends = segment.bounds
        if method == 'max' and np.any(
                np.minimum(ends, segment.frames) <=
                np.minimum(starts, segment.frames)):
            raise IndexError(
                'max(): Expected reduction dim 1 to have non-zero size '
                '(empty word)')
        if method == 'center' and np.any(
                (starts + ends) // 2 >= segment.frames):
            raise IndexError('word center lies beyond the last frame')
```

### emphases_amd/runtime.py

```python
import ctypes
import os

import numpy as np
import torch

HERE = os.path.dirname(os.path.abspath(__file__))
LIBRARY_PATH = os.path.join(HERE, 'libemphases_hip.so')
ABI_VERSION = 38

SEG_FIELDS = 8
TILE_FIELDS = 4
(SEG_AUDIO_OFF, SEG_AUDIO_LEN, SEG_START, SEG_LENGTH, SEG_FRAME_OFF,
 SEG_FRAMES, SEG_WORD_OFF, SEG_WORDS) = range(8)
AXIS_FRAMES, AXIS_WORDS = 0, 1
AXIS_DECODER = 2
ACTIVATIONS = {None: 0, 'none': 0, 'relu': 1, 'gelu': 2, 'silu': 3,
               'leaky_relu': 4}
REDUCTIONS = {'sum': 0, 'average': 1, 'max': 2, 'center': 3}
POSTPROCESS = {None: 0, 'bce': 1, 'mse': 2}
BCE_FORMS = {'bce': 0, 'mse': 1}
AUDIO_F32, AUDIO_PCM16 = 0, 1
SPREAD_IDENTITY, SPREAD_LOG2 = 0, 1
(METRIC_COUNT, METRIC_BCE, METRIC_SQUARED_ERROR, METRIC_COVARIANCE,
 METRIC_SUM_PREDICTED, METRIC_SUMSQ_PREDICTED, METRIC_SUM_TARGET,
 METRIC_SUMSQ_TARGET, METRIC_FIELDS) = range(9)

_c = ctypes
_ptr, _i32, _i64, _f32 = _c.c_void_p, _c.c_int32, _c.c_int64, _c.c_float

SIGNATURES = {
    'emph_abi_version': (_c.c_int, []),
    'emph_last_error': (_c.c_char_p, []),
    'emph_launch_probe': (_c.c_int, [_ptr]),
    'emph_launch_timer_begin': (_c.c_int, [_i32]),
    'emph_launch_timer_count': (_i32, []),
    'emph_launch_timer_end': (_c.c_int, [_ptr, _i32, _ptr]),
    'emph_frontend_table_size': (_i64, []),
    'emph_frontend_table_fill': (_c.c_int, [_ptr]),
    'emph_frontend_block': (_i32, []),
    'emph_logmel': (_c.c_int, [
        _ptr, _i32, _ptr, _ptr, _i32, _ptr, _ptr, _ptr, _ptr, _ptr, _i32, _ptr,
        _i64, _i32, _i32, _ptr, _ptr, _i32, _ptr]),
    'emph_frontend_peak': (_c.c_int, [
        _ptr, _i32, _ptr, _ptr, _i32, _ptr, _ptr, _ptr]),
    'emph_host_gather': (_c.c_int, [_ptr, _ptr, _ptr, _i32, _ptr, _i32]),
    'emph_resample': (_c.c_int, [
        _ptr, _i32, _ptr, _i32, _i64, _ptr, _i32, _i32, _i32, _ptr, _ptr]),
    'emph_pitch_rows': (_c.c_int, [
        _ptr, _ptr, _ptr, _i64, _i32, _i32, _i32, _f32, _f32, _ptr]),
    'emph_conv_pack_size': (_i64, [_i32, _i32, _i32]),
    'emph_conv_pack': (_c.c_int, [_ptr, _i32, _i32, _i32, _ptr]),
    'emph_conv1d': (_c.c_int, [
        _ptr, _i64, _ptr, _i64, _ptr, _ptr, _i32, _i32, _i32, _i32, _ptr, _i32,
        _i32, _i32, _ptr]),
    'emph_conv_winograd_pack_size': (_i64, [_i32, _i32]),
    'emph_conv_winograd_lds_bytes': (_i64, [_i32, _i32]),
    'emph_conv_winograd_pack': (_c.c_int, [_ptr, _i32, _i32, _ptr]),
    'emph_conv1d_winograd': (_c.c_int, [
        _ptr, _i64, _ptr, _i64, _ptr, _ptr, _i32, _i32, _i32, _ptr, _i32, _i32,
        _ptr]),
    'emph_conv_winograd4_pack_size': (_i64, [_i32, _i32]),
    'emph_conv_winograd4_lds_bytes': (_i64, [_i32, _i32]),
    'emph_conv_winograd4_pack': (_c.c_int, [_ptr, _i32, _i32, _ptr]),
    'emph_conv1d_winograd4': (_c.c_int, [
        _ptr, _i64, _ptr, _i64, _ptr, _ptr, _i32, _i32, _i32, _ptr, _i32,
        _ptr]),
    'emph_conv1d_winograd4_position': (_c.c_int, [
        _ptr, _i64, _ptr, _i64, _ptr, _ptr, _i32, _i32, _i32, _ptr, _i32,
        _ptr, _i32, _ptr]),
    'emph_conv1d_winograd4_word_sums': (_c.c_int, [
        _ptr, _i64, _ptr, _i64, _ptr, _ptr, _i32, _i32, _i32, _ptr, _i32,
        _ptr, _ptr]),
    'emph_conv_stack_max_layers': (_i32, []),
    'emph_conv_stack_spans': (_i32, [_ptr, _ptr, _i32, _ptr]),
    'emph_conv1d_stack': (_c.c_int, [
        _ptr, _i64, _ptr, _i64, _ptr, _ptr, _i32, _i32, _ptr, _i32, _ptr,
        _ptr]),
    'emph_conv_split_pack_size': (_i64, []),
    'emph_conv_split_pack': (_c.c_int, [_ptr, _ptr]),
    'emph_conv1d_split': (_c.c_int, [
        _ptr, _i64, _ptr, _i64, _ptr, _ptr, _i32, _i32, _ptr, _i32, _ptr,
        _ptr]),
    'emph_word_sums': (_c.c_int, [
        _ptr, _i64, _ptr, _ptr, _ptr, _ptr, _i64, _i32, _i64, _i32, _ptr]),
    'emph_conv_winograd4_split_pack': (_c.c_int, [_ptr, _i32, _i32, _ptr]),
    'emph_conv1d_winograd4_half': (_c.c_int, [
        _ptr, _i64, _ptr, _i64, _ptr, _ptr, _i32, _i32, _i32, _ptr, _i32,
        _ptr, _i32, _i32, _ptr]),
    'emph_segment_reduce': (_c.c_int, [
        _ptr, _i64, _ptr, _ptr, _i64, _i32, _ptr, _ptr, _i64, _i32, _ptr]),
    'emph_output_layer': (_c.c_int, [
        _ptr, _i64, _ptr, _ptr, _i32, _i32, _ptr, _ptr, _i64, _i32, _i32,
        _ptr, _ptr, _ptr]),
    'emph_linear_chain_pack_size': (_i64, [_i32]),
    'emph_linear_chain_pack': (_c.c_int, [_ptr, _i32, _i32, _ptr]),
    'emph_transformer_block': (_c.c_int, [
        _ptr, _ptr, _i64, _i32, _ptr, _ptr, _c.c_float, _i32, _ptr, _i32,
        _i32, _ptr]),
    'emph_transformer_block_qkv': (_c.c_int, [
        _ptr, _ptr, _i64, _i32, _ptr, _ptr, _c.c_float, _i32, _ptr, _i32,
        _i32, _ptr, _ptr, _ptr]),
    'emph_qkv_projection': (_c.c_int, [
        _ptr, _i64, _ptr, _ptr, _i32, _ptr, _ptr, _ptr, _i32, _i32, _ptr]),
    'emph_linear_split_pack_size': (_i64, [_i32]),
    'emph_linear_split_pack': (_c.c_int, [_ptr, _i32, _ptr]),
    'emph_transformer_block_split': (_c.c_int, [
        _ptr, _ptr, _i64, _i32, _ptr, _i32, _ptr, _c.c_float, _i32, _ptr, _i32,
        _i32, _ptr]),
    'emph_linear_split_pack16_size': (_i64, [_i32]),
    'emph_linear_split_pack16': (_c.c_int, [_ptr, _i32, _ptr]),
    'emph_position_wise_split': (_c.c_int, [
        _ptr, _ptr, _i64, _i32, _i32, _ptr, _ptr, _ptr, _ptr, _i32, _i32,
        _c.c_float, _i32, _ptr, _i32, _i32, _ptr, _ptr, _ptr, _ptr]),
    'emph_transformer_block_qkv_split': (_c.c_int, [
        _ptr, _ptr, _i64, _i32, _i32, _ptr, _ptr, _i32, _i32, _ptr, _ptr,
        _c.c_float, _i32, _ptr, _i32, _i32, _ptr, _ptr, _ptr, _ptr]),
    'emph_qkv_projection_split': (_c.c_int, [
        _ptr, _i64, _ptr, _ptr, _i32, _ptr, _i32, _ptr, _ptr, _i32, _i32,
        _ptr]),
    'emph_qkv_projection_split_images': (_c.c_int, [
        _ptr, _i64, _ptr, _ptr, _i32, _i32, _ptr, _i32, _i32, _ptr, _ptr,
        _i32, _i32, _ptr]),
    'emph_prominence_workspace_floats': (
        _i64, [_i32, _i32, _i64, _i64, _i32]),
    'emph_prominence_forward': (_c.c_int, [
        _ptr, _ptr, _i32, _ptr, _ptr, _i32, _ptr, _i32, _i32, _ptr, _i32, _ptr,
        _ptr, _i64, _i64, _ptr, _ptr, _ptr, _ptr, _ptr, _i32, _ptr]),
    'emph_files_affinity': (_c.c_int, [_ptr, _i32]),
    'emph_files_open': (_c.c_int, [_ptr, _ptr, _i32, _i32, _ptr]),
    'emph_files_close': (None, [_ptr]),
    'emph_files_error': (_c.c_char_p, [_ptr, _i32]),
    'emph_files_sizes': (_c.c_int, [_ptr, _ptr]),
    'emph_files_alignments': (_c.c_int, [
        _ptr, _ptr, _ptr, _ptr, _ptr, _ptr, _ptr, _ptr, _ptr, _ptr]),
    'emph_files_tier_name_bytes': (_i64, [_ptr]),
    'emph_files_read_audio': (_c.c_int, [
        _ptr, _ptr, _ptr, _ptr, _i32, _ptr, _i32]),
    'emph_files_write': (_c.c_int, [
        _ptr, _ptr, _ptr, _ptr, _ptr, _i32, _i32]),
    'emph_files_write_tensors': (_c.c_int, [
        _ptr, _ptr, _ptr, _ptr, _ptr, _i32, _i32]),
    'emph_files_write_tensors_error': (_c.c_char_p, [_i32]),
    'emph_plan_tiles': (_i64, [_ptr, _ptr, _i32, _i32, _i64, _i64, _ptr]),
    'emph_plan_batch': (_c.c_int, [
        _ptr, _ptr, _ptr, _i32, _i64, _i64, _i64, _i64, _ptr, _ptr, _ptr, _ptr,
        _ptr, _ptr, _i64, _ptr, _ptr]),
    'emph_plan_word_sums': (_i64, [
        _ptr, _ptr, _ptr, _i32, _ptr, _ptr, _i64, _ptr, _i64, _i64, _i64,
        _ptr, _ptr, _ptr, _ptr, _i64, _ptr]),
    'emph_gather_columns': (_c.c_int, [
        _ptr, _i64, _ptr, _i64, _i32, _ptr, _i32, _ptr]),
    'emph_collate': (_c.c_int, [
        _ptr, _i64, _ptr, _i64, _ptr, _i32, _i32, _i64, _i64, _ptr, _ptr,
        _ptr]),
    'emph_unpack_rows': (_c.c_int, [_ptr, _i64, _ptr, _i32, _ptr, _ptr]),
    'emph_word_decoder_block': (_i32, [_i32, _i32, _i32]),
    'emph_word_decoder_tiles': (_i32, [_ptr, _ptr, _i32, _i32, _i32, _i32, _ptr]),
    'emph_word_decoder_pack_size': (_i64, [_i32, _i32]),
    'emph_word_decoder_pack': (_c.c_int, [_ptr, _i32, _i32, _ptr]),
    'emph_word_decoder': (_c.c_int, [
        _ptr, _i64, _ptr, _i32, _i32, _ptr, _ptr, _i32, _i32, _i32, _ptr, _ptr,
        _i32, _i32, _ptr, _ptr, _ptr]),
    'emph_add_position': (_c.c_int, [
        _ptr, _i64, _ptr, _i32, _i32, _ptr, _i32, _i32, _ptr]),
    'emph_attention': (_c.c_int, [
        _ptr, _ptr, _ptr, _i64, _i32, _i32, _ptr, _i32, _i32, _ptr, _ptr]),
    'emph_split_kv_bytes': (_i64, [_i64, _i32, _i32, _i32, _i32]),
    'emph_split_kv': (_c.c_int, [
        _ptr, _ptr, _i64, _i32, _i32, _ptr, _i32, _i32, _i32, _ptr, _ptr]),
    'emph_attention_split': (_c.c_int, [
        _ptr, _ptr, _ptr, _i64, _i32, _i32, _ptr, _i32, _i32, _ptr, _i32,
        _ptr]),
    'emph_word_transformer_pack_size': (_i64, [_i32, _i32]),
    'emph_word_transformer_pack': (_c.c_int, [_ptr] * 12 + [_i32, _i32, _ptr]),
    'emph_word_transformer': (_c.c_int, [
        _ptr, _i64, _ptr, _i32, _i32, _i32, _ptr, _i32, _f32, _ptr, _i32, _ptr]),
    'emph_word_metrics': (_c.c_int, [
        _ptr, _ptr, _ptr, _i64, _i32, _f32, _f32, _ptr, _ptr]),
    'emph_word_metrics_grouped': (_c.c_int, [
        _ptr, _ptr, _ptr, _i32, _i32, _i32, _f32, _f32, _ptr, _ptr]),
    'emph_add_layernorm': (_c.c_int, [
        _ptr, _ptr, _ptr, _i64, _i32, _ptr, _ptr, _f32, _i64, _i64, _ptr]),
    'emph_quantile_spreads': (_c.c_int, [
        _ptr, _i64, _ptr, _i64, _i32, _ptr, _ptr, _ptr, _i64, _ptr]),
    'emph_take': (_c.c_int, [_ptr, _ptr, _ptr, _i64, _ptr]),
    'emph_loss_grad': (_c.c_int, [
        _ptr, _ptr, _ptr, _i64, _i64, _i32, _ptr, _ptr, _ptr]),
    'emph_output_layer_backward': (_c.c_int, [
        _ptr, _ptr, _i64, _ptr, _ptr, _i32, _i32, _i64, _ptr, _ptr, _ptr,
        _i64, _ptr]),
    'emph_activation_backward': (_c.c_int, [_ptr, _ptr, _i64, _i32, _ptr]),
    'emph_dropout': (_c.c_int, [
        _ptr, _i64, _i64, _f32, _c.c_uint64, _c.c_uint32, _c.c_uint32, _ptr]),
    'emph_activation_dropout_backward': (_c.c_int, [
        _ptr, _ptr, _i64, _i32, _f32, _ptr]),
    'emph_segment_broadcast': (_c.c_int, [
        _ptr, _i64, _ptr, _ptr, _i64, _i32, _ptr, _ptr, _i32, _i32, _ptr]),
    'emph_conv_weight_grad_parts': (_i32, [_i32]),
    'emph_conv_weight_grad': (_c.c_int, [
        _ptr, _i64, _ptr, _i64, _i32, _i32, _i32, _ptr, _i32, _i32, _ptr,
        _ptr, _ptr, _ptr]),
    'emph_conv_weight_grad_split': (_c.c_int, [
        _ptr, _i64, _ptr, _i64, _i32, _i32, _i32, _ptr, _i32, _i32, _ptr,
        _ptr, _ptr, _ptr]),
    'emph_conv_split_pack_device': (_c.c_int, [_ptr, _ptr, _ptr, _i32, _ptr]),
    'emph_conv_weight_grad_any_workspace': (_i64, [_i32, _i32, _i32, _i32]),
    'emph_conv_weight_grad_any': (_c.c_int, [
        _ptr, _i64, _ptr, _i64, _i32, _i32, _i32, _ptr, _i32, _i32, _ptr,
        _ptr, _ptr, _ptr]),
    'emph_segment_reduce_backward': (_c.c_int, [
        _ptr, _i64, _ptr, _ptr, _i64, _ptr, _ptr, _i64, _i32, _ptr, _ptr,
        _i32, _i32, _ptr]),
    'emph_activation_gradient': (_c.c_int, [_ptr, _ptr, _i64, _i32, _ptr]),
    'emph_adam_step': (_c.c_int, [
        _ptr, _ptr, _ptr, _ptr, _i64, _c.c_double, _c.c_double, _f32, _f32,
        _f32, _ptr]),
}

_library = None


class LibraryError(RuntimeError):
    """The HIP library is missing, stale, or reported an error."""


def library():
    global _library
    if _library is None:
        if not os.path.exists(LIBRARY_PATH):
            raise LibraryError(
                f'{LIBRARY_PATH} not found: build it with '
                '`make -C emphases_amd/csrc` (or `__graft_entry__.build()`). '
                'There is no CPU fallback for the HIP path.')
        lib = ctypes.CDLL(LIBRARY_PATH)
        for name, (restype, argtypes) in SIGNATURES.items():
            try:
                function = getattr(lib, name)
            except AttributeError as error:
                raise LibraryError(
                    f'{LIBRARY_PATH} does not export {name}') from error
            function.restype = restype
            function.argtypes = argtypes
        if lib.emph_abi_version() != ABI_VERSION:
            raise LibraryError(
                f'ABI version {lib.emph_abi_version()} != {ABI_VERSION}; '
                'rebuild the library')
        _library = lib
    return _library




def require_gpu(device=None):
    if not torch.cuda.is_available():
        raise LibraryError(
            'no MI355X/HIP device is visible; the prominence hot path has no '
            'CPU fallback (the CPU restatement lives in oracle/ and is test '
            'infrastructure only)')
    if device is None:
        return torch.device('cuda', torch.cuda.current_device())
    if isinstance(device, int):
        return torch.device('cuda', device)
    return torch.device(device)


def check(status, name):
    if status != 0:
        message = library().emph_last_error().decode('utf-8', 'replace')
        raise LibraryError(f'{name} failed with status {status}: {message}')


def pointer(tensor):
    if tensor is None:
        return None
    if isinstance(tensor, np.ndarray):
        assert tensor.flags['C_CONTIGUOUS']
        return tensor.ctypes.data
    assert tensor.is_contiguous()
    return tensor.data_ptr()


def stream():
    return torch.cuda.current_stream().cuda_stream




class LaunchTimer:

    def __init__(self, capacity=4096):
        self.capacity = int(capacity)
        self.microseconds = np.zeros(0, dtype=np.float32)
        self.launches = 0

    def __enter__(self):
        check(library().emph_launch_timer_begin(self.capacity),
              'emph_launch_timer_begin')
        return self

    def count(self):
        return int(library().emph_launch_timer_count())

    def __exit__(self, kind, value, trace):
        durations = np.zeros(self.capacity, dtype=np.float32)
        seen = _i32(0)
        status = library().emph_launch_timer_end(
            durations.ctypes.data, self.capacity, _c.byref(seen))
        if kind is None:
            check(status, 'emph_launch_timer_end')
        self.launches = int(seen.value)
        self.microseconds = durations[:min(self.launches, self.capacity)]
        return False


def frontend_table():
    lib = library()
    table = np.zeros(lib.emph_frontend_table_size(), dtype=np.float32)
    check(lib.emph_frontend_table_fill(table.ctypes.data),
          'emph_frontend_table_fill')
    return table


def linear_chain_pack(weight, natural):
    lib = library()
    weight = np.ascontiguousarray(weight, dtype=np.float32)
    channels = weight.shape[0]
    assert weight.shape == (channels, channels)
    pack = np.zeros(lib.emph_linear_chain_pack_size(channels),
                    dtype=np.float32)
    check(lib.emph_linear_chain_pack(
        weight.ctypes.data, channels, int(natural), pack.ctypes.data),
        'emph_linear_chain_pack')
    return pack


def word_decoder_tiles(counts, offsets, layers, kernel_size, out_kernel_size):
    lib = library()
    counts = np.ascontiguousarray(counts, dtype=np.int64)
    offsets = np.ascontiguousarray(offsets, dtype=np.int64)
    arguments = (counts.ctypes.data, offsets.ctypes.data, len(counts),
                 int(layers), int(kernel_size), int(out_kernel_size))
    total = lib.emph_word_decoder_tiles(*arguments, None)
    if total < 0:
        raise ValueError('emph_word_decoder_tiles: bad decoder shape')
    tiles = np.zeros((total, TILE_FIELDS), dtype=np.int32)
    if total:
        lib.emph_word_decoder_tiles(*arguments, tiles.ctypes.data)
    return tiles


def word_transformer_pack(state, prefix, channels, heads):
    lib = library()
    names = ('self_attn.in_proj_weight', 'self_attn.in_proj_bias',
             'self_attn.out_proj.weight', 'self_attn.out_proj.bias',
             'linear1.weight', 'linear1.bias', 'linear2.weight', 'linear2.bias',
             'norm1.weight', 'norm1.bias', 'norm2.weight', 'norm2.bias')
    arrays = [np.ascontiguousarray(state[prefix + name], dtype=np.float32)
              for name in names]
    pack = np.zeros(lib.emph_word_transformer_pack_size(channels, heads),
                    dtype=np.float32)
    check(lib.emph_word_transformer_pack(
        *[array.ctypes.data for array in arrays], channels, heads,
        pack.ctypes.data), 'emph_word_transformer_pack')
    return pack


class ConvModel(_c.Structure):
    _fields_ = [(name, _i32) for name in (
        'channels', 'features', 'encoder_layers', 'decoder_layers',
        'decoder_kernel_size', 'activation', 'reduction', 'post',
        'normalize', 'mel_nnz', 'conv_variant')] + [(name, _ptr) for name in (
            'table', 'mel_start', 'mel_count', 'mel_offset', 'mel_values',
            'input_pack', 'input_bias', 'encoder_packs', 'encoder_biases',
            'decoder_packs', 'decoder_biases', 'out_weight', 'out_bias')]


class WordSumTables(_c.Structure):
    _fields_ = [(name, _ptr) for name in (
        'slot_map', 'terms', 'first', 'lengths')] + [('n_slots', _i32)]


def word_decoder_pack(weight):
    lib = library()
    weight = np.ascontiguousarray(weight, dtype=np.float32)
    channels, c_in, kernel_size = weight.shape
    assert channels == c_in
    pack = np.zeros(
        lib.emph_word_decoder_pack_size(channels, kernel_size),
        dtype=np.float32)
    check(lib.emph_word_decoder_pack(
        weight.ctypes.data, channels, kernel_size, pack.ctypes.data),
        'emph_word_decoder_pack')
    return pack


def conv_split_pack(weight):
    lib = library()
    weight = np.ascontiguousarray(weight, dtype=np.float32)
    assert weight.shape == (80, 80, 3)
    pack = np.zeros(lib.emph_conv_split_pack_size(), dtype=np.uint8)
    check(lib.emph_conv_split_pack(weight.ctypes.data, pack.ctypes.data),
          'emph_conv_split_pack')
    return pack


def linear_split_pack(weight, pieces=2, tile=32):
    lib = library()
    weight = np.ascontiguousarray(weight, dtype=np.float32)
    assert weight.shape == (80, 80) and tile in (16, 32)
    size, fill = (lib.emph_linear_split_pack_size, lib.emph_linear_split_pack) \
        if tile == 32 else \
        (lib.emph_linear_split_pack16_size, lib.emph_linear_split_pack16)
    pack = np.zeros(size(pieces), dtype=np.uint8)
    check(fill(weight.ctypes.data, pieces, pack.ctypes.data),
          'emph_linear_split_pack')
    return pack


def conv_winograd4_pack(weight, split=False):
    lib = library()
    weight = np.ascontiguousarray(weight, dtype=np.float32)
    c_out, c_in, kernel_size = weight.shape
    assert kernel_size == 3
    pack = np.zeros(
        lib.emph_conv_winograd4_pack_size(c_out, c_in), dtype=np.float32)
    function = lib.emph_conv_winograd4_split_pack if split else \
        lib.emph_conv_winograd4_pack
    check(function(weight.ctypes.data, c_out, c_in, pack.ctypes.data),
          'emph_conv_winograd4_pack')
    return pack


def conv_winograd4_lds_bytes(c_out, c_in):
    return int(library().emph_conv_winograd4_lds_bytes(c_out, c_in))


def conv_winograd_lds_bytes(c_out, c_in):
    return int(library().emph_conv_winograd_lds_bytes(c_out, c_in))


def conv_winograd_pack(weight):
    lib = library()
    weight = np.ascontiguousarray(weight, dtype=np.float32)
    c_out, c_in, kernel_size = weight.shape
    assert kernel_size == 3
    pack = np.zeros(
        lib.emph_conv_winograd_pack_size(c_out, c_in), dtype=np.float32)
    check(lib.emph_conv_winograd_pack(
        weight.ctypes.data, c_out, c_in, pack.ctypes.data),
        'emph_conv_winograd_pack')
    return pack


def conv_pack(weight):
    lib = library()
    weight = np.ascontiguousarray(weight, dtype=np.float32)
    if weight.ndim == 2:
        weight = weight[:, :, None]
    c_out, c_in, kernel_size = weight.shape
    pack = np.zeros(
        lib.emph_conv_pack_size(c_out, c_in, kernel_size), dtype=np.float32)
    check(lib.emph_conv_pack(
        weight.ctypes.data, c_out, c_in, kernel_size, pack.ctypes.data),
        'emph_conv_pack')
    return pack
```

### include/emphases_hip.h

```cpp
#ifndef EMPHASES_HIP_H
#define EMPHASES_HIP_H

#include <stdint.h>

#ifdef __cplusplus
extern "C" {
#endif

#define EMPH_ABI_VERSION 38

enum {
    EMPH_SEG_AUDIO_OFF = 0,
    EMPH_SEG_AUDIO_LEN = 1,
    EMPH_SEG_START = 2,
    EMPH_SEG_LENGTH = 3,
    EMPH_SEG_FRAME_OFF = 4,
    EMPH_SEG_FRAMES = 5,
    EMPH_SEG_WORD_OFF = 6,
    EMPH_SEG_WORDS = 7,
    EMPH_SEG_FIELDS = 8
};

enum { EMPH_AXIS_FRAMES = 0, EMPH_AXIS_WORDS = 1 };

enum {
    EMPH_TILE_SEGMENT = 0,
    EMPH_TILE_FIRST = 1,
    EMPH_TILE_OFFSET = 2,
    EMPH_TILE_COUNT = 3,
    EMPH_TILE_FIELDS = 4
};

enum {
    EMPH_ACT_NONE = 0,
    EMPH_ACT_RELU = 1,
    EMPH_ACT_GELU = 2,
    EMPH_ACT_SILU = 3,
    EMPH_ACT_LEAKY_RELU = 4
};

enum {
    EMPH_REDUCE_SUM = 0,
    EMPH_REDUCE_AVERAGE = 1,
    EMPH_REDUCE_MAX = 2,
    EMPH_REDUCE_CENTER = 3
};

enum { EMPH_AUDIO_F32 = 0, EMPH_AUDIO_PCM16 = 1 };

enum { EMPH_POST_NONE = 0, EMPH_POST_SIGMOID = 1, EMPH_POST_CLAMP01 = 2 };

enum {
    EMPH_OK = 0,
    EMPH_EINVAL = -1,
    EMPH_ERANGE = -2
};

int emph_abi_version(void);
const char* emph_last_error(void);


int emph_host_gather(const void* const* host_sources, const int64_t* host_bytes,
                     const int64_t* host_offsets, int32_t count,
                     void* host_destination, int32_t threads);


typedef struct emph_file_batch emph_file_batch;

int emph_files_affinity(const int32_t* cpus, int32_t count);

int emph_files_open(const char* const* text_paths,
                    const char* const* audio_paths, int32_t count,
                    int32_t threads, emph_file_batch** batch);
void emph_files_close(emph_file_batch* batch);
const char* emph_files_error(const emph_file_batch* batch, int32_t index);

int emph_files_sizes(const emph_file_batch* batch, int64_t* sizes);

int emph_files_alignments(const emph_file_batch* batch, double* word_times,
                          char* word_text, int64_t* word_text_end,
                          double* phone_times, char* phone_text,
                          int64_t* phone_text_end, int32_t* phone_word,
                          char* tier_names, int64_t* tier_names_end);
int64_t emph_files_tier_name_bytes(const emph_file_batch* batch);

int emph_files_read_audio(const emph_file_batch* batch, const int32_t* which,
                          const int64_t* where, const int64_t* bytes,
                          int32_t count, void* destination, int32_t threads);

int emph_files_write(const emph_file_batch* batch, const int32_t* which,
                     const char* const* prefixes, const float* scores,
                     const int64_t* first, int32_t count, int32_t threads);

int emph_files_write_tensors(const char* const* paths, const float* data,
                             const int64_t* first, const int64_t* rows,
                             const int64_t* columns, int32_t count,
                             int32_t threads);
const char* emph_files_write_tensors_error(int32_t index);

int64_t emph_plan_tiles(const int64_t* host_counts, const int64_t* host_offsets,
                        int32_t n_segments, int32_t block, int64_t least,
                        int64_t most, int32_t* host_tiles);
int emph_plan_batch(const double* times, const int64_t* counts,
                    const int64_t* lengths, int32_t n_utterances,
                    int64_t sample_rate, int64_t hopsize, int64_t padding,
                    int64_t num_fft, int64_t* utterance, int64_t* start_sample,
                    int64_t* length, int64_t* frames, int64_t* words,
                    int64_t* bounds, int64_t capacity, int64_t* n_segments,
                    int64_t* n_words);
int64_t emph_plan_word_sums(const int64_t* frames, const int64_t* frame_off,
                            const int64_t* words, int32_t n_segments,
                            const int64_t* word_columns, const int64_t* bounds,
                            int64_t total_words, const int64_t* restarts,
                            int64_t n_restarts, int64_t ld_frames,
                            int64_t ld_words, int32_t* slot_map, int32_t* first,
                            int32_t* lengths, int32_t* terms, int64_t capacity,
                            int32_t* n_slots);


int64_t emph_frontend_table_size(void);

int32_t emph_frontend_block(void);

int emph_frontend_table_fill(float* host_table);

int emph_logmel(const void* audio, int32_t audio_format, const int64_t* seg,
                const int32_t* tiles, int32_t n_tiles, const float* table,
                const int32_t* mel_start, const int32_t* mel_count,
                const int32_t* mel_offset, const float* mel_values,
                int32_t mel_nnz, float* out, int64_t ld, int32_t mel_row,
                int32_t loud_row, const float* seg_peak,
                const float* a_weights, int32_t normalize, void* stream);

int emph_frontend_peak(const void* audio, int32_t audio_format,
                       const int64_t* seg, const int32_t* tiles,
                       int32_t n_tiles, const float* table, float* seg_peak,
                       void* stream);

int emph_resample(const void* audio, int32_t audio_format, const int64_t* table,
                  int32_t n_utterances, int64_t most_samples,
                  const float* kernel, int32_t orig, int32_t fresh,
                  int32_t width, float* out, void* stream);

int emph_pitch_rows(const float* pitch, const float* periodicity, float* out,
                    int64_t ld, int32_t pitch_row, int32_t periodicity_row,
                    int32_t normalize, float logfmin, float logfmax,
                    void* stream);


int64_t emph_conv_pack_size(int32_t c_out, int32_t c_in, int32_t kernel_size);

int emph_conv_pack(const float* host_weight, int32_t c_out, int32_t c_in,
                   int32_t kernel_size, float* host_pack);

int emph_conv1d(const float* x, int64_t ldx, float* y, int64_t ldy,
                const float* pack, const float* bias, int32_t c_in,
                int32_t c_out, int32_t kernel_size, int32_t activation,
                const int32_t* tiles, int32_t n_tiles, int32_t tile_n,
                int32_t transpose_out, void* stream);

int64_t emph_conv_winograd_pack_size(int32_t c_out, int32_t c_in);
int64_t emph_conv_winograd_lds_bytes(int32_t c_out, int32_t c_in);
int emph_conv_winograd_pack(const float* host_weight, int32_t c_out,
                            int32_t c_in, float* host_pack);
int emph_conv1d_winograd(const float* x, int64_t ldx, float* y, int64_t ldy,
                         const float* pack, const float* bias, int32_t c_in,
                         int32_t c_out, int32_t activation,
                         const int32_t* tiles, int32_t n_tiles, int32_t tile_n,
                         void* stream);

int64_t emph_conv_winograd4_pack_size(int32_t c_out, int32_t c_in);
int64_t emph_conv_winograd4_lds_bytes(int32_t c_out, int32_t c_in);
int emph_conv_winograd4_pack(const float* host_weight, int32_t c_out,
                             int32_t c_in, float* host_pack);
int emph_conv1d_winograd4(const float* x, int64_t ldx, float* y, int64_t ldy,
                          const float* pack, const float* bias, int32_t c_in,
                          int32_t c_out, int32_t activation,
                          const int32_t* tiles, int32_t n_tiles, void* stream);
int emph_conv1d_winograd4_position(const float* x, int64_t ldx, float* y,
                                   int64_t ldy, const float* pack,
                                   const float* bias, int32_t c_in,
                                   int32_t c_out, int32_t activation,
                                   const int32_t* tiles, int32_t n_tiles,
                                   const float* position,
                                   int32_t max_positions, void* stream);

int emph_conv1d_winograd4_word_sums(const float* x, int64_t ldx, float* sums,
                                    int64_t ld_sums, const float* pack,
                                    const float* bias, int32_t c_in,
                                    int32_t c_out, int32_t activation,
                                    const int32_t* tiles, int32_t n_tiles,
                                    const int32_t* slot_map, void* stream);

int32_t emph_conv_stack_max_layers(void);
int32_t emph_conv_stack_spans(const int64_t* host_counts,
                              const int64_t* host_offsets, int32_t n_segments,
                              int32_t* host_spans);
int emph_conv1d_stack(const float* x, int64_t ldx, float* y, int64_t ldy,
                      const float* packs, const float* biases, int32_t layers,
                      int32_t relu_mask, const int32_t* spans, int32_t n_spans,
                      const int32_t* slot_map, void* stream);

int64_t emph_conv_split_pack_size(void);
int emph_conv_split_pack(const float* host_weight, void* host_pack);
int emph_conv1d_split(const float* x, int64_t ldx, float* y, int64_t ldy,
                      const void* packs, const float* biases, int32_t layers,
                      int32_t relu_mask, const int32_t* spans, int32_t n_spans,
                      const int32_t* slot_map, void* stream);

int emph_conv_winograd4_split_pack(const float* host_weight, int32_t c_out,
                                   int32_t c_in, float* host_pack);
int emph_conv1d_winograd4_half(const float* x, int64_t ldx, float* y,
                               int64_t ldy, const float* split_pack,
                               const float* bias, int32_t c_in, int32_t c_out,
                               int32_t activation, const int32_t* tiles,
                               int32_t n_tiles, const float* position,
                               int32_t max_positions, int32_t half,
                               void* stream);


int emph_segment_reduce(const float* x, int64_t ldx, const int32_t* bounds,
                        float* out, int64_t ldw, int32_t channels,
                        const int64_t* seg, const int32_t* word_segment,
                        int64_t total_words, int32_t mode, void* stream);

int emph_word_sums(const float* sums, int64_t ld_sums, const int32_t* terms,
                   const int32_t* first, const int32_t* lengths, float* out,
                   int64_t ldw, int32_t channels, int64_t columns, int32_t mode,
                   void* stream);


int emph_output_layer(const float* x, int64_t ldx, const float* weight,
                      const float* bias, int32_t channels,
                      int32_t kernel_size, const int64_t* seg,
                      const int32_t* position_segment, int64_t total,
                      int32_t axis, int32_t post, float* logits,
                      float* scores, void* stream);

int emph_gather_columns(const float* x, int64_t ldx, float* y, int64_t ldy,
                        int32_t channels, const int64_t* pieces,
                        int32_t n_pieces, void* stream);

int emph_collate(const float* features, int64_t ld_cache, const float* targets,
                 int64_t total_words, const int64_t* items, int32_t n_items,
                 int32_t channels, int64_t ld_frames, int64_t ld_words,
                 float* out_features, float* out_targets, void* stream);

int emph_unpack_rows(const float* x, int64_t ld, const int64_t* table,
                     int32_t n, float* out, void* stream);


int32_t emph_word_decoder_block(int32_t layers, int32_t kernel_size,
                                int32_t out_kernel_size);

int32_t emph_word_decoder_tiles(const int64_t* host_counts,
                                const int64_t* host_offsets, int32_t segments,
                                int32_t layers, int32_t kernel_size,
                                int32_t out_kernel_size, int32_t* host_tiles);

int64_t emph_word_decoder_pack_size(int32_t channels, int32_t kernel_size);
int emph_word_decoder_pack(const float* host_weight, int32_t channels,
                           int32_t kernel_size, float* host_pack);

int emph_word_decoder(const float* x, int64_t ldx, const int32_t* tiles,
                      int32_t n_tiles, int32_t channels, const float* packs,
                      const float* biases, int32_t layers, int32_t kernel_size,
                      int32_t activation, const float* out_weight,
                      const float* out_bias, int32_t out_kernel_size,
                      int32_t post, float* logits, float* scores, void* stream);


int emph_add_position(float* x, int64_t ldx, const float* table,
                      int32_t channels, int32_t max_positions,
                      const int32_t* tiles, int32_t n_tiles, int32_t tile_n,
                      void* stream);

int emph_attention(const float* qk, const float* v, float* out, int64_t ld,
                   int32_t channels, int32_t heads, const int32_t* tiles,
                   int32_t n_tiles, int32_t tile_n, const int32_t* key_counts,
                   void* stream);

int64_t emph_split_kv_bytes(int64_t ld, int32_t n_segments, int32_t channels,
                            int32_t heads, int32_t pieces);
int emph_split_kv(const float* qk, const float* v, int64_t ld, int32_t channels,
                  int32_t heads, const int32_t* tiles, int32_t n_tiles,
                  int32_t tile_n, int32_t pieces, void* images, void* stream);
int emph_attention_split(const float* qk, const void* images, float* out,
                         int64_t ld, int32_t channels, int32_t heads,
                         const int32_t* tiles, int32_t n_tiles, int32_t tile_n,
                         const int32_t* key_counts, int32_t pieces, void* stream);

int emph_add_layernorm(const float* x, const float* r, float* y, int64_t ld,
                       int32_t channels, const float* gamma,
                       const float* beta, float eps, int64_t first_column,
                       int64_t columns, void* stream);

int64_t emph_linear_chain_pack_size(int32_t channels);
int emph_linear_chain_pack(const float* host_weight, int32_t channels,
                           int32_t natural, float* host_pack);
int emph_transformer_block(const float* attended, float* x, int64_t ld,
                           int32_t channels, const float* packs,
                           const float* vectors, float eps, int32_t activation,
                           const int32_t* tiles, int32_t n_tiles,
                           int32_t tile_n, void* stream);

int emph_transformer_block_qkv(const float* attended, float* x, int64_t ld,
                               int32_t channels, const float* packs,
                               const float* vectors, float eps,
                               int32_t activation, const int32_t* tiles,
                               int32_t n_tiles, int32_t tile_n, float* qk,
                               float* v, void* stream);

int emph_qkv_projection(const float* x, int64_t ld, float* qk, float* v,
                        int32_t channels, const float* packs,
                        const float* bias, const int32_t* tiles,
                        int32_t n_tiles, int32_t tile_n, void* stream);

int64_t emph_linear_split_pack_size(int32_t pieces);
int emph_linear_split_pack(const float* host_weight , int32_t pieces,
                           void* host_pack);
int emph_transformer_block_split(const float* attended, float* x, int64_t ld,
                                 int32_t channels, const void* packs,
                                 int32_t pieces, const float* vectors, float eps,
                                 int32_t activation, const int32_t* tiles,
                                 int32_t n_tiles, int32_t tile_n, void* stream);
int emph_qkv_projection_split(const float* x, int64_t ld, float* qk, float* v,
                              int32_t channels, const void* packs,
                              int32_t pieces, const float* bias,
                              const int32_t* tiles, int32_t n_tiles,
                              int32_t tile_n, void* stream);
int emph_transformer_block_qkv_split(const float* attended, float* x, int64_t ld,
                                     int32_t channels, int32_t heads,
                                     const void* block_packs, const void* qkv_packs,
                                     int32_t pieces, int32_t attention_pieces,
                                     const float* vectors, const float* qkv_bias,
                                     float eps, int32_t activation,
                                     const int32_t* tiles, int32_t n_tiles,
                                     int32_t tile_n, float* qk, float* v,
                                     void* images, void* stream);
int64_t emph_linear_split_pack16_size(int32_t pieces);
int emph_linear_split_pack16(const float* host_weight , int32_t pieces,
                             void* host_pack);
int emph_position_wise_split(const float* attended, float* x, int64_t ld,
                             int32_t channels, int32_t heads, const void* block_packs,
                             const float* vectors, const void* qkv_packs,
                             const float* qkv_bias, int32_t pieces,
                             int32_t attention_pieces, float eps, int32_t activation,
                             const int32_t* tiles, int32_t n_tiles, int32_t tile_n,
                             float* qk, float* v, void* images, void* stream);
int emph_qkv_projection_split_images(const float* x, int64_t ld, float* qk,
                                     void* images, int32_t channels,
                                     int32_t heads, const void* packs,
                                     int32_t pieces, int32_t attention_pieces,
                                     const float* bias, const int32_t* tiles,
                                     int32_t n_tiles, int32_t tile_n,
                                     void* stream);

int64_t emph_word_transformer_pack_size(int32_t channels, int32_t heads);
int emph_word_transformer_pack(
    const float* in_proj_weight, const float* in_proj_bias,
    const float* out_weight, const float* out_bias,
    const float* linear1_weight, const float* linear1_bias,
    const float* linear2_weight, const float* linear2_bias,
    const float* norm1_weight, const float* norm1_bias,
    const float* norm2_weight, const float* norm2_bias, int32_t channels,
    int32_t heads, float* host_pack);
int emph_word_transformer(float* x, int64_t ld, const float* position,
                          int32_t max_positions, int32_t channels,
                          int32_t heads, const float* packs, int32_t layers,
                          float eps, const int32_t* tiles, int32_t n_tiles,
                          void* stream);


enum {
    EMPH_METRIC_COUNT = 0,
    EMPH_METRIC_BCE = 1,
    EMPH_METRIC_SQUARED_ERROR = 2,
    EMPH_METRIC_COVARIANCE = 3,
    EMPH_METRIC_SUM_PREDICTED = 4,
    EMPH_METRIC_SUMSQ_PREDICTED = 5,
    EMPH_METRIC_SUM_TARGET = 6,
    EMPH_METRIC_SUMSQ_TARGET = 7,
    EMPH_METRIC_FIELDS = 8
};

int emph_word_metrics(const float* logits, const float* targets,
                      const int32_t* word_segment, int64_t total, int32_t post,
                      float predicted_mean, float target_mean,
                      double* accumulators, void* stream);

enum {
    EMPH_BCE_WITH_LOGITS = 0,
    EMPH_BCE_CLAMPED_LOG = 1
};

int emph_word_metrics_grouped(const float* logits, const float* targets,
                              const int64_t* cu_words, int32_t groups,
                              int32_t post, int32_t bce_form,
                              float predicted_mean, float target_mean,
                              double* out, void* stream);


enum {
    EMPH_SPREAD_IDENTITY = 0,
    EMPH_SPREAD_LOG2 = 1
};

int emph_quantile_spreads(const float* values, int64_t ld, const int64_t* segments,
                          int64_t n_segments, int32_t transform, float* stats,
                          float* selected, float* out, int64_t n_rows,
                          void* stream);


typedef struct emph_conv_model {
    int32_t channels;
    int32_t features;
    int32_t encoder_layers;
    int32_t decoder_layers;
    int32_t decoder_kernel_size;
    int32_t activation;
    int32_t reduction;
    int32_t post;
    int32_t normalize;
    int32_t mel_nnz;
    int32_t conv_variant;
    const float* table;
    const int32_t* mel_start;
    const int32_t* mel_count;
    const int32_t* mel_offset;
    const float* mel_values;
    const float* input_pack;
    const float* input_bias;
    const float* encoder_packs;
    const float* encoder_biases;
    const float* decoder_packs;
    const float* decoder_biases;
    const float* out_weight;
    const float* out_bias;
} emph_conv_model;

typedef struct emph_word_sum_tables {
    const int32_t* slot_map;
    const int32_t* terms;
    const int32_t* first;
    const int32_t* lengths;
    int32_t n_slots;
} emph_word_sum_tables;

int64_t emph_prominence_workspace_floats(int32_t features, int32_t channels,
                                         int64_t ld_frames, int64_t ld_words,
                                         int32_t n_slots);

int emph_prominence_forward(const emph_conv_model* model, const void* audio,
                            int32_t audio_format, const int64_t* seg,
                            const int32_t* frontend_tiles,
                            int32_t n_frontend_tiles,
                            const int32_t* frame_tiles, int32_t n_frame_tiles,
                            int32_t tile_n, const int32_t* word_tiles,
                            int32_t n_word_tiles, const int32_t* bounds,
                            const int32_t* word_segment, int64_t ld_frames,
                            int64_t ld_words, float* workspace, float* logits,
                            float* scores,
                            const emph_word_sum_tables* word_sums,
                            const int32_t* conv_spans, int32_t n_conv_spans,
                            void* stream);



int emph_take(const float* src, const int32_t* index, float* out, int64_t count,
              void* stream);

int emph_loss_grad(const float* logits, const float* targets,
                   const int32_t* word_segment, int64_t columns, int64_t valid_words,
                   int32_t form, float* loss, float* dlogit, void* stream);

int emph_output_layer_backward(const float* dlogit, const float* x, int64_t ldx,
                               const float* weight, const int32_t* word_segment,
                               int32_t channels, int32_t kernel_size, int64_t columns,
                               float* dweight, float* dbias, float* dx, int64_t ld_dx,
                               void* stream);

int emph_activation_backward(const float* y, float* gradient, int64_t count,
                             int32_t activation, void* stream);

int emph_dropout(float* x, int64_t count, int64_t origin, float p, uint64_t seed,
                 uint32_t stream_id, uint32_t step, void* stream);
int emph_activation_dropout_backward(const float* y, float* gradient, int64_t count,
                                     int32_t activation, float p, void* stream);

int emph_segment_broadcast(const float* dword, int64_t ldw, const int32_t* bounds,
                           float* dx, int64_t ldx, int32_t channels, const int64_t* seg,
                           const int32_t* tiles, int32_t n_tiles, int32_t mode,
                           void* stream);

int32_t emph_conv_weight_grad_parts(int32_t n_tiles);
int emph_conv_weight_grad(const float* dy, int64_t ld_dy, const float* x, int64_t ldx,
                          int32_t c_in, int32_t c_out, int32_t kernel_size,
                          const int32_t* tiles, int32_t n_tiles, int32_t tile_n,
                          float* workspace, float* dweight, float* dbias, void* stream);

int emph_conv_weight_grad_split(const float* dy, int64_t ld_dy, const float* x, int64_t ldx,
                                int32_t c_in, int32_t c_out, int32_t kernel_size,
                                const int32_t* tiles, int32_t n_tiles, int32_t tile_n,
                                float* workspace, float* dweight, float* dbias,
                                void* stream);
int emph_conv_split_pack_device(const float* weights, const int32_t* index, void* packs,
                                int32_t count, void* stream);

int emph_adam_step(float* parameter, const float* gradient, float* exp_avg,
                   float* exp_avg_sq, int64_t count, double beta1, double beta2,
                   float step_size, float correction2_sqrt, float eps, void* stream);


int64_t emph_conv_weight_grad_any_workspace(int32_t c_in, int32_t c_out, int32_t kernel_size,
                                            int32_t n_tiles);
int emph_conv_weight_grad_any(const float* dy, int64_t ld_dy, const float* x, int64_t ldx,
                              int32_t c_in, int32_t c_out, int32_t kernel_size,
                              const int32_t* tiles, int32_t n_tiles, int32_t tile_n,
                              float* workspace, float* dweight, float* dbias, void* stream);

int emph_segment_reduce_backward(const float* dword, int64_t ldw, const int32_t* bounds,
                                 const float* x, int64_t ldx, const float* y, float* dx,
                                 int64_t ld_dx, int32_t channels, const int64_t* seg,
                                 const int32_t* tiles, int32_t n_tiles, int32_t mode,
                                 void* stream);

int emph_activation_gradient(const float* source, float* gradient, int64_t count,
                             int32_t activation, void* stream);


int emph_launch_probe(void* stream);

int emph_launch_timer_begin(int32_t capacity);
int32_t emph_launch_timer_count(void);
int emph_launch_timer_end(float* host_microseconds, int32_t capacity, int32_t* host_count);

#ifdef __cplusplus
}
#endif
#endif
```

Baseline: 435,800 utterances/s.

## Compose input conv and first encoder conv into one width-5 convolution

Since there is no activation between the input layer and the first encoder layer, the two k=3 convolutions are folded on the host into one k=5 convolution with combined bias. The first layer of the fused stack kernel then runs an 8-point transform variant that uses 2-step weight chunks. A separate edge correction is computed at the utterance boundaries, where the intermediate zero padding breaks the composition. This removes one full 80x80 conv layer of work and its weight streaming, in exchange for more points per step in the composed layer, extra edge-fixup logic and new loader scheduling.

```diff
diff --git a/emphases_amd/csrc/conv_stack.hip b/emphases_amd/csrc/conv_stack.hip
--- a/emphases_amd/csrc/conv_stack.hip
+++ b/emphases_amd/csrc/conv_stack.hip
@@ -24,20 +24,34 @@
 constexpr int kStackMaxLayers = 3;
 constexpr int kSpanFields = 8;
 
+constexpr int kComposePoints = 8;
+constexpr int kComposeChunkSteps = 2;
+constexpr int kComposeChunks = kStackSteps / kComposeChunkSteps;
+constexpr int kComposeStepFloats = kComposePoints * kStackMTiles * 64;
+constexpr int kComposeChunkFloats = kComposeChunkSteps * kComposeStepFloats;
+constexpr int kComposePackFloats = kStackSteps * kComposeStepFloats;
+constexpr int kComposeBias = kComposePackFloats;
+constexpr int kComposeEdge = kComposeBias + kStackChannels;
+constexpr int kComposeEdgeFloats = kStackChannels * kStackChannels + kStackChannels;
+constexpr int kComposeFloats = kComposeEdge + 2 * kComposeEdgeFloats;
+static_assert(kComposeChunkFloats <= kStackChunkFloats, "a composed chunk fits a ring slot");
+
 __host__ __device__ constexpr int stack_lds_floats() {
     return kStackChannels * kStackStride + 2 * kStackChunkFloats +
-           kStackMaxLayers * kStackChannels;
-}
-
-template <bool WORD_SUMS>
+           kStackMaxLayers * kStackChannels + 2 * kStackChannels;
+}
+
+template <bool WORD_SUMS, bool COMPOSE>
 __global__ __launch_bounds__(kStackThreads) void conv1d_stack_kernel(
     const float* __restrict__ x, int64_t ldx, float* __restrict__ y, int64_t ldy,
     const float* __restrict__ packs, const float* __restrict__ biases, int layers,
-    int relu_mask, const int32_t* __restrict__ spans, const int32_t* __restrict__ slot_map) {
+    int relu_mask, const int32_t* __restrict__ spans, const int32_t* __restrict__ slot_map,
+    const float* __restrict__ compose) {
     extern __shared__ __align__(16) float lds[];
     float* act = lds;
     float* ring = act + kStackChannels * kStackStride;
     float* bias_lds = ring + 2 * kStackChunkFloats;
+    float* edge_lds = bias_lds + kStackMaxLayers * kStackChannels;
     const int lane = threadIdx.x & 63;
     const int wave = __builtin_amdgcn_readfirstlane(threadIdx.x >> 6);
     const bool loader = wave >= 8;
@@ -51,21 +65,31 @@
     const int c0 = span_b.y;
 
     constexpr int kPackFloats = kStackSteps * kStackStepFloats;
-    const int total_chunks = layers * kStackChunks;
+    constexpr int kFirstChunks = COMPOSE ? kComposeChunks : 0;
+    const int total_chunks = COMPOSE ? kFirstChunks + (layers - 1) * kStackChunks
+                                     : layers * kStackChunks;
     auto request = [&](int g, int first, int n) {
-        const int layer = g / kStackChunks;
-        const float* source = packs + static_cast<int64_t>(layer) * kPackFloats +
-                              (g - layer * kStackChunks) * kStackChunkFloats;
+        const bool composed = COMPOSE && g < kFirstChunks;
+        const int layer = (g - kFirstChunks) / kStackChunks;
+        const float* source =
+            composed ? compose + g * kComposeChunkFloats
+                     : packs + static_cast<int64_t>(layer) * kPackFloats +
+                           (g - kFirstChunks - layer * kStackChunks) * kStackChunkFloats;
         float* target = ring + (g & 1) * kStackChunkFloats;
-        constexpr int kQuads = kStackChunkFloats / 4;
-        const int each = (kQuads / 64 + n - 1) / n;
+        const int quads = (composed ? kComposeChunkFloats : kStackChunkFloats) / 4;
+        const int each = (quads / 64 + n - 1) / n;
         for (int k = 0; k < each; ++k) {
-            const int from = min(((wave - first) + k * n) * 64, kQuads - 64);
+            const int from = min(((wave - first) + k * n) * 64, quads - 64);
             __builtin_amdgcn_global_load_lds(
                 (const __attribute__((address_space(1))) void*)(source + 4 * (from + lane)),
                 (__attribute__((address_space(3))) void*)(target + 4 * from), 16, 0, 0);
         }
     };
+    auto layer_starts = [&](int g) {
+        return COMPOSE ? g >= kFirstChunks && (g - kFirstChunks) % kStackChunks == 0
+                       : g % kStackChunks == 0;
+    };
+    constexpr int kShift = COMPOSE ? 2 : 1;
     STACK_STAMP(0);
 
     const int last_quad = (count - 1) & ~3;
@@ -85,9 +109,23 @@
     auto deposit = [&](int c, int q, const float4& raw) {
         const float4 v = masked(q, raw);
         float* target = act + c * kStackStride + 4 * q;
-        target[1] = v.x;
-        *reinterpret_cast<f32x2*>(target + 2) = f32x2{v.y, v.z};
-        target[4] = v.w;
+        if (COMPOSE) {
+            *reinterpret_cast<f32x2*>(target + 2) = f32x2{v.x, v.y};
+            *reinterpret_cast<f32x2*>(target + 4) = f32x2{v.z, v.w};
+        } else {
+            target[1] = v.x;
+            *reinterpret_cast<f32x2*>(target + 2) = f32x2{v.y, v.z};
+            target[4] = v.w;
+        }
+    };
+    auto side_index = [&](int kind) {
+        return COMPOSE ? (kind < 2 ? kind : kStackWidth + kind)
+                       : (kind == 0 ? 0 : kStackWidth + kind);
+    };
+    auto side_position = [&](int kind) { return c0 - kShift + side_index(kind); };
+    auto side_is_real = [&](int kind) {
+        const int p = side_position(kind);
+        return (COMPOSE || kind < 3) && p >= 0 && p < count;
     };
     constexpr int kEarlyRows = 16;
     if (loader) {
@@ -101,15 +139,14 @@
         const float* source = x + static_cast<int64_t>(mine >> 6) * ldx + column + min(p, last_quad);
         const uint32_t target = static_cast<uint32_t>(reinterpret_cast<uintptr_t>(
             (__attribute__((address_space(3))) float*)(act + (mine >> 6) * kStackStride + 4 * q)));
-        const int side_kind = mine < 64 ? (mine & 3) : 3;
-        const int side_p = side_kind == 0 ? c0 - 1 : c0 + kStackWidth + side_kind - 1;
-        const bool side_real = side_kind < 3 && side_p >= 0 && side_p < count;
+        const int side_kind = (COMPOSE || mine < 64) ? (mine & 3) : 3;
+        const int side_p = side_position(side_kind);
+        const bool side_real = side_is_real(side_kind);
         const float* side_source = x + static_cast<int64_t>((mine >> 2) & 15) * ldx + column +
                                    (side_real ? side_p : 0);
         const uint32_t side_target = static_cast<uint32_t>(reinterpret_cast<uintptr_t>(
             (__attribute__((address_space(3))) float*)(
-                act + ((mine >> 2) & 15) * kStackStride +
-                (side_kind == 0 ? 0 : kStackWidth + side_kind))));
+                act + ((mine >> 2) & 15) * kStackStride + side_index(side_kind))));
         auto ask = [&](int chunk) {
 #pragma unroll
             for (int round = 0; round < kStage; ++round) {
@@ -128,13 +165,23 @@
                 const f32x2 middle = {p + 1 < count ? raw[1] : 0.f, p + 2 < count ? raw[2] : 0.f};
                 const float last = p + 3 < count ? raw[3] : 0.f;
                 const uint32_t address = target + (16 * chunk + 4 * round) * (kStackStride * 4);
-                asm volatile(
-                    "ds_write_b32 %0, %1 offset:4\n\t"
-                    "ds_write_b64 %0, %2 offset:8\n\t"
-                    "ds_write_b32 %0, %3 offset:16"
-                    :
-                    : "v"(address), "v"(first), "v"(middle), "v"(last)
-                    : "memory");
+                if (COMPOSE) {
+                    const f32x2 left = {first, middle[0]}, right = {middle[1], last};
+                    asm volatile(
+                        "ds_write_b64 %0, %1 offset:8\n\t"
+                        "ds_write_b64 %0, %2 offset:16"
+                        :
+                        : "v"(address), "v"(left), "v"(right)
+                        : "memory");
+                } else {
+                    asm volatile(
+                        "ds_write_b32 %0, %1 offset:4\n\t"
+                        "ds_write_b64 %0, %2 offset:8\n\t"
+                        "ds_write_b32 %0, %3 offset:16"
+                        :
+                        : "v"(address), "v"(first), "v"(middle), "v"(last)
+                        : "memory");
+                }
             }
             const float beside = side_real ? side[chunk - 1] : 0.f;
             const uint32_t address = side_target + 16 * chunk * (kStackStride * 4);
@@ -144,6 +191,31 @@
     asm volatile("s_waitcnt vmcnt(" #COUNT ")"                                              \
                  : "+v"(rows[STAGE][0]), "+v"(rows[STAGE][1]), "+v"(rows[STAGE][2]),        \
                    "+v"(rows[STAGE][3]), "+v"(side[STAGE])::"memory")
+        if (COMPOSE) {
+            request(1, 8, 4);
+            ask(1);
+            __builtin_amdgcn_s_barrier();
+            ask(2);
+            EMPH_ROWS_HERE(5, 0);
+            hand_over(1);
+            asm volatile("s_waitcnt lgkmcnt(0)" ::: "memory");
+            __builtin_amdgcn_s_barrier();
+            request(2, 8, 4);
+            ask(3);
+            EMPH_ROWS_HERE(5, 1);
+            hand_over(2);
+            asm volatile("s_waitcnt lgkmcnt(0)" ::: "memory");
+            __builtin_amdgcn_s_barrier();
+            request(3, 8, 4);
+            ask(4);
+            EMPH_ROWS_HERE(5, 2);
+            hand_over(3);
+            asm volatile("s_waitcnt lgkmcnt(0)" ::: "memory");
+            __builtin_amdgcn_s_barrier();
+            request(4, 8, 4);
+            EMPH_ROWS_HERE(5, 3);
+            hand_over(4);
+        } else {
         request(1, 8, 4);
         ask(1);
         __builtin_amdgcn_s_barrier();
@@ -167,13 +239,42 @@
         request(4, 8, 4);
         EMPH_ROWS_HERE(8, 3);
         hand_over(4);
+        }
 #undef EMPH_ROWS_HERE
+        const int edge_side = mine >> 7, edge_channel = mine & 127;
+        const int last_index = count - 1 - c0;
+        const bool edge_mine = COMPOSE && edge_channel < kStackChannels &&
+                               (edge_side ? last_index >= 0 && last_index < kStackWidth : c0 == 0);
+        const float* edge_matrix = compose + kComposeEdge + edge_side * kComposeEdgeFloats + edge_channel;
+        const float* edge_x = act + kShift + (edge_side ? last_index : 0);
+        float edge_value = 0.f;
         for (int g = 4; g < total_chunks; ++g) {
             asm volatile("s_waitcnt vmcnt(0) lgkmcnt(0)" ::: "memory");
-            STACK_STAMP(2 + 8 * (g / kStackChunks) + g % kStackChunks);
+            STACK_STAMP(COMPOSE && g < kFirstChunks
+                            ? 2 + (g >> 1)
+                            : 2 + 8 * ((g - kFirstChunks / 2) / kStackChunks) +
+                                  (g - kFirstChunks) % kStackChunks);
             __syncthreads();
+            constexpr int kPiece = 16;
+            const bool piece = edge_mine && g < 4 + kStackChannels / kPiece;
+            float edge_weights[kPiece];
+            if (piece) {
+                const int row = (g - 4) * kPiece;
+                if (g == 4) edge_value = edge_matrix[kStackChannels * kStackChannels];
+#pragma unroll
+                for (int i = 0; i < kPiece; ++i)
+                    edge_weights[i] = edge_matrix[(row + i) * kStackChannels];
+            }
             if (g + 1 < total_chunks) request(g + 1, 8, 4);
-            if ((g + 1) % kStackChunks == 0 && g + 1 < total_chunks) __syncthreads();
+            if (piece) {
+                const int row = (g - 4) * kPiece;
+#pragma unroll
+                for (int i = 0; i < kPiece; ++i)
+                    edge_value = fmaf(edge_weights[i], edge_x[(row + i) * kStackStride], edge_value);
+                if (g == 3 + kStackChannels / kPiece)
+                    edge_lds[edge_side * kStackChannels + edge_channel] = edge_value;
+            }
+            if (layer_starts(g + 1) && g + 1 < total_chunks) __syncthreads();
         }
         return;
     }
@@ -181,7 +282,10 @@
     {
         static_assert(kStackMaxLayers * kStackChannels <= 512, "one bias per thread");
         const bool has_bias = threadIdx.x < layers * kStackChannels;
-        const float bias_value = has_bias ? biases[threadIdx.x] : 0.f;
+        const int bias_index = COMPOSE ? static_cast<int>(threadIdx.x) - kStackChannels : threadIdx.x;
+        const float bias_value = !has_bias ? 0.f
+                                 : bias_index < 0 ? compose[kComposeBias + threadIdx.x]
+                                                  : biases[bias_index];
         constexpr int kEarly = kEarlyRows * 64 / 512;
         float4 early[kEarly];
 #pragma unroll
@@ -193,8 +297,7 @@
         const int side_row = threadIdx.x >> 2, side_kind = threadIdx.x & 3;
         if (side_row < kEarlyRows) {
             const float* row = x + static_cast<int64_t>(side_row) * ldx + column;
-            const int p = side_kind == 0 ? c0 - 1 : c0 + kStackWidth + side_kind - 1;
-            if (side_kind < 3 && p >= 0 && p < count) side = row[p];
+            if (side_is_real(side_kind)) side = row[side_position(side_kind)];
         }
 #pragma unroll
         for (int round = 0; round < kEarly; ++round) {
@@ -202,7 +305,7 @@
             deposit(index >> 6, index & 63, early[round]);
         }
         if (side_row < kEarlyRows)
-            act[side_row * kStackStride + (side_kind == 0 ? 0 : kStackWidth + side_kind)] = side;
+            act[side_row * kStackStride + side_index(side_kind)] = side;
         if (has_bias) bias_lds[threadIdx.x] = bias_value;
     }
     STACK_STAMP(1);
@@ -218,57 +321,86 @@
 
     auto run = [&](auto count_tag) {
         constexpr int COUNT = decltype(count_tag)::value;
-        for (int layer = 0; layer < layers; ++layer) {
-            f32x4 acc[6][COUNT];
-#pragma unroll
-            for (int j = 0; j < 6; ++j)
+        auto run_layer = [&](int layer, auto points_tag) {
+            constexpr int POINTS = decltype(points_tag)::value;
+            constexpr bool FIVE = POINTS == kComposePoints;
+            constexpr int kSteps = FIVE ? kComposeChunkSteps : kStackChunkSteps;
+            constexpr int kChunks = kStackSteps / kSteps;
+            const int first_chunk =
+                COMPOSE ? (layer == 0 ? 0 : kFirstChunks + (layer - 1) * kStackChunks)
+                        : layer * kStackChunks;
+            f32x4 acc[POINTS][COUNT];
+#pragma unroll
+            for (int j = 0; j < POINTS; ++j)
 #pragma unroll
                 for (int m = 0; m < COUNT; ++m) acc[j][m] = f32x4{0.f, 0.f, 0.f, 0.f};
-            float a[6][COUNT], d[6], v[6];
+            float a[POINTS][COUNT], d[POINTS], v[POINTS];
             auto load_b = [&](int step) {
                 const float* source = lane_rows + 4 * step * kStackStride;
                 const f32x4 first = *reinterpret_cast<const f32x4*>(source);
-                const f32x2 second = *reinterpret_cast<const f32x2*>(source + 4);
                 d[0] = first[0], d[1] = first[1], d[2] = first[2], d[3] = first[3];
-                d[4] = second[0], d[5] = second[1];
+                if constexpr (FIVE) {
+                    const f32x4 second = *reinterpret_cast<const f32x4*>(source + 4);
+                    d[4] = second[0], d[5] = second[1], d[6] = second[2], d[7] = second[3];
+                } else {
+                    const f32x2 second = *reinterpret_cast<const f32x2*>(source + 4);
+                    d[4] = second[0], d[5] = second[1];
+                }
             };
-            for (int chunk = 0; chunk < kStackChunks; ++chunk) {
+            for (int chunk = 0; chunk < kChunks; ++chunk) {
                 __syncthreads();
-                STACK_STAMP(2 + 8 * layer + chunk);
-                if (chunk == 0 || layer == 0) load_b(chunk * kStackChunkSteps);
+                STACK_STAMP(FIVE ? 2 + (chunk >> 1)
+                                 : 2 + 8 * layer + chunk);
+                if (chunk == 0 || layer == 0) load_b(chunk * kSteps);
                 const float* weights =
-                    ring + ((layer * kStackChunks + chunk) & 1) * kStackChunkFloats +
-                    (m_begin << 6) + lane;
-#pragma unroll
-                for (int ks = 0; ks < kStackChunkSteps; ++ks) {
-                    const int step = chunk * kStackChunkSteps + ks;
-#pragma unroll
-                    for (int j = 0; j < 6; ++j)
+                    ring + ((first_chunk + chunk) & 1) * kStackChunkFloats + (m_begin << 6) + lane;
+#pragma unroll
+                for (int ks = 0; ks < kSteps; ++ks) {
+                    const int step = chunk * kSteps + ks;
+#pragma unroll
+                    for (int j = 0; j < POINTS; ++j)
 #pragma unroll
                         for (int m = 0; m < COUNT; ++m)
 #ifdef STACK_FEWER_A_READS
                             a[j][m] = (j & 1) ? a[j - 1][m]
-                                              : weights[(ks * 6 * kStackMTiles + j * kStackMTiles + m) << 6];
+                                              : weights[(ks * POINTS * kStackMTiles + j * kStackMTiles + m) << 6];
 #else
-                            a[j][m] = weights[(ks * 6 * kStackMTiles + j * kStackMTiles + m) << 6];
+                            a[j][m] = weights[(ks * POINTS * kStackMTiles + j * kStackMTiles + m) << 6];
 #endif
 #ifdef STACK_NO_TRANSFORM
-                    for (int j = 0; j < 6; ++j) v[j] = d[j];
+                    for (int j = 0; j < POINTS; ++j) v[j] = d[j];
 #else
-                    const float p = fmaf(-4.f, d[2], d[4]);
-                    const float q = fmaf(-4.f, d[1], d[3]);
-                    const float c = d[4] - d[2];
-                    const float e = 2.f * (d[3] - d[1]);
-                    v[0] = fmaf(4.f, d[0], fmaf(-5.f, d[2], d[4]));
-                    v[1] = p + q;
-                    v[2] = p - q;
-                    v[3] = c + e;
-                    v[4] = c - e;
-                    v[5] = fmaf(4.f, d[1], fmaf(-5.f, d[3], d[5]));
+                    if constexpr (FIVE) {
+                        const float even1 = fmaf(-4.25f, d[4], d[2] + d[6]);
+                        const float odd1 = fmaf(-4.25f, d[3], d[1] + d[5]);
+                        const float even2 = fmaf(0.25f, d[2], fmaf(-1.25f, d[4], d[6]));
+                        const float odd2 = fmaf(0.5f, d[1], fmaf(-2.5f, d[3], 2.f * d[5]));
+                        const float even3 = fmaf(4.f, d[2], fmaf(-5.f, d[4], d[6]));
+                        const float odd3 = fmaf(2.f, d[1], fmaf(-2.5f, d[3], 0.5f * d[5]));
+                        v[0] = fmaf(5.25f, d[4] - d[2], d[0] - d[6]);
+                        v[1] = even1 + odd1;
+                        v[2] = even1 - odd1;
+                        v[3] = even2 + odd2;
+                        v[4] = even2 - odd2;
+                        v[5] = even3 + odd3;
+                        v[6] = even3 - odd3;
+                        v[7] = fmaf(5.25f, d[3] - d[5], d[7] - d[1]);
+                    } else {
+                        const float p = fmaf(-4.f, d[2], d[4]);
+                        const float q = fmaf(-4.f, d[1], d[3]);
+                        const float c = d[4] - d[2];
+                        const float e = 2.f * (d[3] - d[1]);
+                        v[0] = fmaf(4.f, d[0], fmaf(-5.f, d[2], d[4]));
+                        v[1] = p + q;
+                        v[2] = p - q;
+                        v[3] = c + e;
+                        v[4] = c - e;
+                        v[5] = fmaf(4.f, d[1], fmaf(-5.f, d[3], d[5]));
+                    }
 #endif
                     if (step + 1 < kStackSteps) load_b(step + 1);
 #pragma unroll
-                    for (int j = 0; j < 6; ++j)
+                    for (int j = 0; j < POINTS; ++j)
 #pragma unroll
                         for (int m = 0; m < COUNT; ++m)
                             acc[j][m] = __builtin_amdgcn_mfma_f32_16x16x4f32(
@@ -278,28 +410,53 @@
             const bool relu = (relu_mask >> layer) & 1;
             const bool last = layer == layers - 1;
             const float* bias_row = bias_lds + layer * kStackChannels;
-            STACK_STAMP(2 + 8 * layer + 5);
+            auto outputs = [&](int m, int r, int channel, float add, float& o0, float& o1,
+                               float& o2, float& o3) {
+                const float m1 = acc[1][m][r], m2 = acc[2][m][r];
+                const float m3 = acc[3][m][r], m4 = acc[4][m][r];
+                const float s12 = m1 + m2, d12 = m1 - m2, s34 = m3 + m4, d34 = m3 - m4;
+                if constexpr (FIVE) {
+                    const float m5 = acc[5][m][r], m6 = acc[6][m][r];
+                    const float s56 = m5 + m6, d56 = m5 - m6;
+                    o0 = acc[0][m][r] + s12 + s34 + s56 + add;
+                    o1 = fmaf(0.5f, d56, fmaf(2.f, d34, d12)) + add;
+                    o2 = fmaf(0.25f, s56, fmaf(4.f, s34, s12)) + add;
+                    o3 = fmaf(0.125f, d56, fmaf(8.f, d34, d12)) + acc[7][m][r] + add;
+                    const float left = edge_lds[channel];
+                    const float right = edge_lds[kStackChannels + channel];
+                    const int at = count - 1 - p_quad;
+                    o0 -= p_quad == 0 ? left : 0.f;
+                    o0 -= at == 0 ? right : 0.f;
+                    o1 -= at == 1 ? right : 0.f;
+                    o2 -= at == 2 ? right : 0.f;
+                    o3 -= at == 3 ? right : 0.f;
+                } else {
+                    o0 = acc[0][m][r] + s12 + s34 + add;
+                    o1 = fmaf(2.f, d34, d12) + add;
+                    o2 = fmaf(4.f, s34, s12) + add;
+                    o3 = fmaf(8.f, d34, d12) + acc[5][m][r] + add;
+                }
+                if (relu) {
+                    o0 = o0 < 0.f ? 0.f : o0;
+                    o1 = o1 < 0.f ? 0.f : o1;
+                    o2 = o2 < 0.f ? 0.f : o2;
+                    o3 = o3 < 0.f ? 0.f : o3;
+                }
+            };
+            STACK_STAMP(FIVE ? 7 : 2 + 8 * layer + 5);
             if (!last) {
                 __syncthreads();
+                if (FIVE && threadIdx.x < kStackChannels)
+                    act[threadIdx.x * kStackStride + kStackWidth + 1] =
+                        act[threadIdx.x * kStackStride + kStackWidth + 2];
 #pragma unroll
                 for (int m = 0; m < COUNT; ++m) {
                     const int channel0 = 16 * (m_begin + m) + 4 * kk;
                     const f32x4 add = *reinterpret_cast<const f32x4*>(bias_row + channel0);
 #pragma unroll
                     for (int r = 0; r < 4; ++r) {
-                        const float m1 = acc[1][m][r], m2 = acc[2][m][r];
-                        const float m3 = acc[3][m][r], m4 = acc[4][m][r];
-                        const float s12 = m1 + m2, d12 = m1 - m2, s34 = m3 + m4, d34 = m3 - m4;
-                        float o0 = acc[0][m][r] + s12 + s34 + add[r];
-                        float o1 = fmaf(2.f, d34, d12) + add[r];
-                        float o2 = fmaf(4.f, s34, s12) + add[r];
-                        float o3 = fmaf(8.f, d34, d12) + acc[5][m][r] + add[r];
-                        if (relu) {
-                            o0 = o0 < 0.f ? 0.f : o0;
-                            o1 = o1 < 0.f ? 0.f : o1;
-                            o2 = o2 < 0.f ? 0.f : o2;
-                            o3 = o3 < 0.f ? 0.f : o3;
-                        }
+                        float o0, o1, o2, o3;
+                        outputs(m, r, channel0 + r, add[r], o0, o1, o2, o3);
                         o0 = p_quad < count ? o0 : 0.f;
                         o1 = p_quad + 1 < count ? o1 : 0.f;
                         o2 = p_quad + 2 < count ? o2 : 0.f;
@@ -311,8 +468,8 @@
                         target[3] = o3;
                     }
                 }
-                STACK_STAMP(2 + 8 * layer + 6);
-                continue;
+                STACK_STAMP(FIVE ? 8 : 2 + 8 * layer + 6);
+                return;
             }
             const int t = p_quad;
             const int owned_end = owned_first + owned;
@@ -326,19 +483,8 @@
                     f32x4 sum[4];
 #pragma unroll
                     for (int r = 0; r < 4; ++r) {
-                        const float m1 = acc[1][m][r], m2 = acc[2][m][r];
-                        const float m3 = acc[3][m][r], m4 = acc[4][m][r];
-                        const float s12 = m1 + m2, d12 = m1 - m2, s34 = m3 + m4, d34 = m3 - m4;
-                        float o0 = acc[0][m][r] + s12 + s34 + add[r];
-                        float o1 = fmaf(2.f, d34, d12) + add[r];
-                        float o2 = fmaf(4.f, s34, s12) + add[r];
-                        float o3 = fmaf(8.f, d34, d12) + acc[5][m][r] + add[r];
-                        if (relu) {
-                            o0 = o0 < 0.f ? 0.f : o0;
-                            o1 = o1 < 0.f ? 0.f : o1;
-                            o2 = o2 < 0.f ? 0.f : o2;
-                            o3 = o3 < 0.f ? 0.f : o3;
-                        }
+                        float o0, o1, o2, o3;
+                        outputs(m, r, channel0 + r, add[r], o0, o1, o2, o3);
                         o0 = (t >= owned_first && t < owned_end) ? o0 : 0.f;
                         o1 = (t + 1 >= owned_first && t + 1 < owned_end) ? o1 : 0.f;
                         o2 = (t + 2 >= owned_first && t + 2 < owned_end) ? o2 : 0.f;
@@ -369,7 +515,7 @@
                                                       channel0) = sum[j];
                     }
                 }
-                continue;
+                return;
             }
             const bool vector_ok = (ldy & 3) == 0 && (column & 3) == 0 &&
                                    (reinterpret_cast<uintptr_t>(y) & 15) == 0;
@@ -379,20 +525,8 @@
                 const f32x4 add = *reinterpret_cast<const f32x4*>(bias_row + channel0);
 #pragma unroll
                 for (int r = 0; r < 4; ++r) {
-                    const float m1 = acc[1][m][r], m2 = acc[2][m][r];
-                    const float m3 = acc[3][m][r], m4 = acc[4][m][r];
-                    const float s12 = m1 + m2, d12 = m1 - m2, s34 = m3 + m4, d34 = m3 - m4;
                     float4 out;
-                    out.x = acc[0][m][r] + s12 + s34 + add[r];
-                    out.y = fmaf(2.f, d34, d12) + add[r];
-                    out.z = fmaf(4.f, s34, s12) + add[r];
-                    out.w = fmaf(8.f, d34, d12) + acc[5][m][r] + add[r];
-                    if (relu) {
-                        out.x = out.x < 0.f ? 0.f : out.x;
-                        out.y = out.y < 0.f ? 0.f : out.y;
-                        out.z = out.z < 0.f ? 0.f : out.z;
-                        out.w = out.w < 0.f ? 0.f : out.w;
-                    }
+                    outputs(m, r, channel0 + r, add[r], out.x, out.y, out.z, out.w);
                     float* target = y + static_cast<int64_t>(channel0 + r) * ldy + column + t;
                     if (vector_ok && t >= owned_first && t + 3 < owned_end) {
                         *reinterpret_cast<float4*>(target) = out;
@@ -404,8 +538,11 @@
                     }
                 }
             }
-            STACK_STAMP(2 + 8 * layer + 6);
-        }
+            STACK_STAMP(FIVE ? 8 : 2 + 8 * layer + 6);
+        };
+        if constexpr (COMPOSE) run_layer(0, std::integral_constant<int, kComposePoints>{});
+        for (int layer = COMPOSE ? 1 : 0; layer < layers; ++layer)
+            run_layer(layer, std::integral_constant<int, 6>{});
     };
     if (part == 0) run(std::integral_constant<int, split>{});
     else run(std::integral_constant<int, kStackMTiles - split>{});
@@ -467,6 +604,35 @@
     return total;
 }
 
+static int launch_stack(const char* name, const float* x, int64_t ldx, float* y, int64_t ldy,
+                        const float* compose, const float* packs, const float* biases,
+                        int32_t layers, int32_t relu_mask, const int32_t* spans, int32_t n_spans,
+                        const int32_t* slot_map, void* stream) {
+    EMPH_REQUIRE(layers >= 1 && layers <= kStackMaxLayers, EMPH_ERANGE,
+                 "%s: %d layers (1 .. %d)", name, layers, kStackMaxLayers);
+    EMPH_REQUIRE((reinterpret_cast<uintptr_t>(x) & 15) == 0 && (ldx & 3) == 0, EMPH_EINVAL,
+                 "%s: the input must be 16-byte aligned with ldx a multiple of 4", name);
+    EMPH_REQUIRE(slot_map == nullptr ||
+                     ((reinterpret_cast<uintptr_t>(y) & 15) == 0 && (ldy & 3) == 0 &&
+                      ldy >= kStackChannels && (reinterpret_cast<uintptr_t>(slot_map) & 15) == 0),
+                 EMPH_EINVAL, "%s: bad sums buffer or slot map", name);
+    const size_t lds = static_cast<size_t>(stack_lds_floats()) * sizeof(float);
+    hipStream_t s = static_cast<hipStream_t>(stream);
+    auto launch = [&](auto kernel, LdsReservation& reserved) {
+        if (int status = reserve_lds(reserved, reinterpret_cast<const void*>(kernel), lds, name))
+            return status;
+        EMPH_LAUNCH(kernel, dim3(n_spans), dim3(kStackThreads), lds, s, x, ldx, y, ldy, packs,
+                    biases, layers, relu_mask, spans, slot_map, compose);
+        return check_launch(name);
+    };
+    static LdsReservation reserved[4];
+    if (compose != nullptr)
+        return slot_map != nullptr ? launch(conv1d_stack_kernel<true, true>, reserved[3])
+                                   : launch(conv1d_stack_kernel<false, true>, reserved[2]);
+    return slot_map != nullptr ? launch(conv1d_stack_kernel<true, false>, reserved[1])
+                               : launch(conv1d_stack_kernel<false, false>, reserved[0]);
+}
+
 int emph_conv1d_stack(const float* x, int64_t ldx, float* y, int64_t ldy, const float* packs,
                       const float* biases, int32_t layers, int32_t relu_mask,
                       const int32_t* spans, int32_t n_spans, const int32_t* slot_map,
@@ -474,34 +640,87 @@
     if (n_spans == 0) return EMPH_OK;
     EMPH_REQUIRE(x && y && packs && biases && spans, EMPH_EINVAL,
                  "emph_conv1d_stack: null pointer");
-    EMPH_REQUIRE(layers >= 1 && layers <= kStackMaxLayers, EMPH_ERANGE,
-                 "emph_conv1d_stack: %d layers (1 .. %d)", layers, kStackMaxLayers);
-    EMPH_REQUIRE((reinterpret_cast<uintptr_t>(x) & 15) == 0 && (ldx & 3) == 0, EMPH_EINVAL,
-                 "emph_conv1d_stack: the input must be 16-byte aligned with ldx a multiple of 4");
-    EMPH_REQUIRE(slot_map == nullptr ||
-                     ((reinterpret_cast<uintptr_t>(y) & 15) == 0 && (ldy & 3) == 0 &&
-                      ldy >= kStackChannels && (reinterpret_cast<uintptr_t>(slot_map) & 15) == 0),
-                 EMPH_EINVAL, "emph_conv1d_stack: bad sums buffer or slot map");
-    const size_t lds = static_cast<size_t>(stack_lds_floats()) * sizeof(float);
-    hipStream_t s = static_cast<hipStream_t>(stream);
-    if (slot_map != nullptr) {
-        auto kernel = conv1d_stack_kernel<true>;
-        static LdsReservation reserved;
-        if (int status = reserve_lds(reserved, reinterpret_cast<const void*>(kernel), lds,
-                                     "emph_conv1d_stack"))
-            return status;
-        EMPH_LAUNCH(kernel, dim3(n_spans), dim3(kStackThreads), lds, s, x, ldx, y, ldy, packs,
-                    biases, layers, relu_mask, spans, slot_map);
-    } else {
-        auto kernel = conv1d_stack_kernel<false>;
-        static LdsReservation reserved;
-        if (int status = reserve_lds(reserved, reinterpret_cast<const void*>(kernel), lds,
-                                     "emph_conv1d_stack"))
-            return status;
-        EMPH_LAUNCH(kernel, dim3(n_spans), dim3(kStackThreads), lds, s, x, ldx, y, ldy, packs,
-                    biases, layers, relu_mask, spans, slot_map);
+    return launch_stack("emph_conv1d_stack", x, ldx, y, ldy, nullptr, packs, biases, layers,
+                        relu_mask, spans, n_spans, slot_map, stream);
+}
+
+int64_t emph_conv_compose_pack_size(void) { return kComposeFloats; }
+
+int emph_conv_compose_pack(const float* w0, const float* b0, const float* w1, const float* b1,
+                           float* host_pack) {
+    EMPH_REQUIRE(w0 && b0 && w1 && b1 && host_pack, EMPH_EINVAL,
+                 "emph_conv_compose_pack: null pointer");
+    constexpr int C = kStackChannels;
+    static const double G[8][5] = {
+        {1., 0., 0., 0., 0.},
+        {-2. / 9, -2. / 9, -2. / 9, -2. / 9, -2. / 9},
+        {-2. / 9, 2. / 9, -2. / 9, 2. / 9, -2. / 9},
+        {1. / 90, 1. / 45, 2. / 45, 4. / 45, 8. / 45},
+        {1. / 90, -1. / 45, 2. / 45, -4. / 45, 8. / 45},
+        {32. / 45, 16. / 45, 8. / 45, 4. / 45, 2. / 45},
+        {32. / 45, -16. / 45, 8. / 45, -4. / 45, 2. / 45},
+        {0., 0., 0., 0., 1.}};
+    auto at = [](const float* w, int o, int i, int k) {
+        return static_cast<double>(w[(o * C + i) * 3 + k]);
+    };
+    double* wc = static_cast<double*>(malloc(sizeof(double) * C * C * 5));
+    EMPH_REQUIRE(wc != nullptr, EMPH_EINVAL, "emph_conv_compose_pack: out of memory");
+    for (int o = 0; o < C; ++o)
+        for (int i = 0; i < C; ++i)
+            for (int d = 0; d < 5; ++d) {
+                double sum = 0.;
+                for (int a = 0; a < 3; ++a) {
+                    const int c = d - a;
+                    if (c < 0 || c > 2) continue;
+                    for (int mid = 0; mid < C; ++mid) sum += at(w1, o, mid, a) * at(w0, mid, i, c);
+                }
+                wc[(o * C + i) * 5 + d] = sum;
+            }
+    for (int step = 0; step < kStackSteps; ++step)
+        for (int j = 0; j < kComposePoints; ++j)
+            for (int m = 0; m < kStackMTiles; ++m)
+                for (int lane = 0; lane < 64; ++lane) {
+                    const double* w = wc + ((16 * m + (lane & 15)) * C + 4 * step + (lane >> 4)) * 5;
+                    double value = 0.;
+                    for (int d = 0; d < 5; ++d) value += G[j][d] * w[d];
+                    host_pack[(((step * kComposePoints + j) * kStackMTiles + m) << 6) + lane] =
+                        static_cast<float>(value);
+                }
+    free(wc);
+    for (int o = 0; o < C; ++o) {
+        double sum = b1[o];
+        for (int mid = 0; mid < C; ++mid)
+            sum += (at(w1, o, mid, 0) + at(w1, o, mid, 1) + at(w1, o, mid, 2)) * b0[mid];
+        host_pack[kComposeBias + o] = static_cast<float>(sum);
     }
-    return check_launch("emph_conv1d_stack");
-}
-
-}
+    for (int side = 0; side < 2; ++side) {
+        float* edge = host_pack + kComposeEdge + side * kComposeEdgeFloats;
+        const int a = side ? 2 : 0, c = side ? 0 : 2;
+        for (int o = 0; o < C; ++o) {
+            double constant = 0.;
+            for (int mid = 0; mid < C; ++mid) constant += at(w1, o, mid, a) * b0[mid];
+            edge[C * C + o] = static_cast<float>(constant);
+            for (int i = 0; i < C; ++i) {
+                double sum = 0.;
+                for (int mid = 0; mid < C; ++mid) sum += at(w1, o, mid, a) * at(w0, mid, i, c);
+                edge[i * C + o] = static_cast<float>(sum);
+            }
+        }
+    }
+    return EMPH_OK;
+}
+
+int emph_conv1d_stack_composed(const float* x, int64_t ldx, float* y, int64_t ldy,
+                               const float* compose, const float* packs, const float* biases,
+                               int32_t layers, int32_t relu_mask, const int32_t* spans,
+                               int32_t n_spans, const int32_t* slot_map, void* stream) {
+    if (n_spans == 0) return EMPH_OK;
+    EMPH_REQUIRE(x && y && compose && spans && (layers <= 1 || (packs && biases)), EMPH_EINVAL,
+                 "emph_conv1d_stack_composed: null pointer");
+    EMPH_REQUIRE((reinterpret_cast<uintptr_t>(compose) & 15) == 0, EMPH_EINVAL,
+                 "emph_conv1d_stack_composed: the composed pack must be 16-byte aligned");
+    return launch_stack("emph_conv1d_stack_composed", x, ldx, y, ldy, compose, packs, biases,
+                        layers, relu_mask, spans, n_spans, slot_map, stream);
+}
+
+}
diff --git a/emphases_amd/csrc/forward.hip b/emphases_amd/csrc/forward.hip
--- a/emphases_amd/csrc/forward.hip
+++ b/emphases_amd/csrc/forward.hip
@@ -84,7 +84,9 @@
                        m.encoder_biases == m.input_bias + c &&
                        (m.activation == EMPH_ACT_RELU || m.activation == EMPH_ACT_NONE);
     if (stack) {
-        const int total = 1 + m.encoder_layers;
+        const bool composed = m.compose != nullptr && m.encoder_layers >= 1;
+        const int skip = composed ? 1 : 0;
+        const int total = 1 + m.encoder_layers - skip;
         const int most = emph_conv_stack_max_layers();
         const int groups = (total + most - 1) / most;
         float* buffers[2] = {current, other};
@@ -94,14 +96,19 @@
             const int size = (total - done + (groups - group) - 1) / (groups - group);
             int relu = 0;
             for (int l = 0; l < size; ++l)
-                if (done + l >= 1 && m.activation == EMPH_ACT_RELU) relu |= 1 << l;
+                if (done + l + skip >= 1 && m.activation == EMPH_ACT_RELU) relu |= 1 << l;
             const bool to_sums = group == groups - 1 && fold;
             float* out = to_sums ? sums : buffers[group & 1];
-            status = emph_conv1d_stack(in, ld_frames, out, to_sums ? c : ld_frames,
-                                       m.input_pack + done * pack_floats,
-                                       m.input_bias + static_cast<int64_t>(done) * c, size, relu,
-                                       conv_spans, n_conv_spans,
-                                       to_sums ? word_sums->slot_map : nullptr, stream);
+            const float* packs = m.input_pack + (done + skip) * pack_floats;
+            const float* biases = m.input_bias + static_cast<int64_t>(done + skip) * c;
+            status = composed && group == 0
+                         ? emph_conv1d_stack_composed(
+                               in, ld_frames, out, to_sums ? c : ld_frames, m.compose,
+                               packs + pack_floats, biases + c, size, relu, conv_spans,
+                               n_conv_spans, to_sums ? word_sums->slot_map : nullptr, stream)
+                         : emph_conv1d_stack(in, ld_frames, out, to_sums ? c : ld_frames, packs,
+                                             biases, size, relu, conv_spans, n_conv_spans,
+                                             to_sums ? word_sums->slot_map : nullptr, stream);
             if (status) return status;
             in = out;
             done += size;
diff --git a/emphases_amd/engine.py b/emphases_amd/engine.py
--- a/emphases_amd/engine.py
+++ b/emphases_amd/engine.py
@@ -219,6 +219,17 @@
         if self.split_conv:
             self._split_packs = to(np.concatenate(
                 [runtime.conv_split_pack(layer.weight) for layer in frame_stack]))
+        self.compose = bool(
+            self.stack and not self.split_conv and
+            len(self.frame_encoder) > 0 and
+            config.downsample_method in ('sum', 'average') and
+            os.environ.get('EMPHASES_CONV_COMPOSE', '1') != '0')
+        self._compose_pack = None
+        if self.compose:
+            first = self.frame_encoder[0]
+            self._compose_pack = to(runtime.conv_compose_pack(
+                self.input_layer.weight, self.input_layer.bias.cpu().numpy(),
+                first.weight, first.bias.cpu().numpy()))
         self.model = self._conv_model()
 
     def lane(self):
@@ -274,7 +285,8 @@
             decoder_packs=pointer(self.decoder_packs),
             decoder_biases=pointer(self.decoder_biases),
             out_weight=pointer(self.output_weight),
-            out_bias=pointer(self.output_bias))
+            out_bias=pointer(self.output_bias),
+            compose=pointer(self._compose_pack if self.stack else None))
 
     def _stack(self, prefix):
         config, state, dev = self.config, self.state, self.device
@@ -856,7 +868,8 @@
         config = self.config
         channels = config.channels
         spans, span_size = meta['conv_spans']
-        total = 1 + len(self.frame_encoder)
+        skip = int(self.compose)
+        total = 1 + len(self.frame_encoder) - skip
         most = int(self.lib.emph_conv_stack_max_layers())
         groups = -(-total // most)
         fold = 'word_sum_tables' in meta
@@ -872,10 +885,11 @@
         for group in range(groups if frames else 0):
             size = -(-(total - done) // (groups - group))
             relu = sum(1 << l for l in range(size)
-                       if done + l >= 1 and relu_layers)
+                       if done + l + skip >= 1 and relu_layers)
             to_sums = fold and group == groups - 1
             target = sums if to_sums else buffers[group & 1]
-            flops = 2. * 80 * 80 * 3 * plan.total_frames * size
+            flops = 2. * 80 * 80 * 3 * plan.total_frames * (
+                size + (skip if group == 0 else 0))
             if self.split_conv:
                 with self._timed('conv1d_split_frames_80x80_k3', flops):
                     runtime.check(self.lib.emph_conv1d_split(
@@ -889,15 +903,29 @@
                 source = target
                 done += size
                 continue
+            layer = done + skip
             with self._timed('conv1d_stack_frames_80x80_k3', flops):
-                runtime.check(self.lib.emph_conv1d_stack(
-                    source.data_ptr(), ld_f, target.data_ptr(),
-                    channels if to_sums else ld_f,
-                    self._stack_packs[done * pack:].data_ptr(),
-                    self._stack_biases[done * channels:].data_ptr(), size,
-                    relu, spans.data_ptr(), span_size // 8,
-                    view('slot_map').data_ptr() if to_sums else None,
-                    runtime.stream()), 'emph_conv1d_stack')
+                if self.compose and group == 0:
+                    runtime.check(self.lib.emph_conv1d_stack_composed(
+                        source.data_ptr(), ld_f, target.data_ptr(),
+                        channels if to_sums else ld_f,
+                        self._compose_pack.data_ptr(),
+                        self._stack_packs[(layer + 1) * pack:].data_ptr()
+                        if size > 1 else None,
+                        self._stack_biases[(layer + 1) * channels:].data_ptr()
+                        if size > 1 else None, size,
+                        relu, spans.data_ptr(), span_size // 8,
+                        view('slot_map').data_ptr() if to_sums else None,
+                        runtime.stream()), 'emph_conv1d_stack_composed')
+                else:
+                    runtime.check(self.lib.emph_conv1d_stack(
+                        source.data_ptr(), ld_f, target.data_ptr(),
+                        channels if to_sums else ld_f,
+                        self._stack_packs[layer * pack:].data_ptr(),
+                        self._stack_biases[layer * channels:].data_ptr(),
+                        size, relu, spans.data_ptr(), span_size // 8,
+                        view('slot_map').data_ptr() if to_sums else None,
+                        runtime.stream()), 'emph_conv1d_stack')
             source = target
             done += size
         if not words:
diff --git a/emphases_amd/runtime.py b/emphases_amd/runtime.py
--- a/emphases_amd/runtime.py
+++ b/emphases_amd/runtime.py
@@ -6,7 +6,7 @@
 
 HERE = os.path.dirname(os.path.abspath(__file__))
 LIBRARY_PATH = os.path.join(HERE, 'libemphases_hip.so')
-ABI_VERSION = 38
+ABI_VERSION = 39
 
 SEG_FIELDS = 8
 TILE_FIELDS = 4
@@ -76,6 +76,11 @@
     'emph_conv1d_stack': (_c.c_int, [
         _ptr, _i64, _ptr, _i64, _ptr, _ptr, _i32, _i32, _ptr, _i32, _ptr,
         _ptr]),
+    'emph_conv_compose_pack_size': (_i64, []),
+    'emph_conv_compose_pack': (_c.c_int, [_ptr, _ptr, _ptr, _ptr, _ptr]),
+    'emph_conv1d_stack_composed': (_c.c_int, [
+        _ptr, _i64, _ptr, _i64, _ptr, _ptr, _ptr, _i32, _i32, _ptr, _i32,
+        _ptr, _ptr]),
     'emph_conv_split_pack_size': (_i64, []),
     'emph_conv_split_pack': (_c.c_int, [_ptr, _ptr]),
     'emph_conv1d_split': (_c.c_int, [
@@ -372,7 +377,8 @@
         'normalize', 'mel_nnz', 'conv_variant')] + [(name, _ptr) for name in (
             'table', 'mel_start', 'mel_count', 'mel_offset', 'mel_values',
             'input_pack', 'input_bias', 'encoder_packs', 'encoder_biases',
-            'decoder_packs', 'decoder_biases', 'out_weight', 'out_bias')]
+            'decoder_packs', 'decoder_biases', 'out_weight', 'out_bias',
+            'compose')]
 
 
 class WordSumTables(_c.Structure):
@@ -394,6 +400,19 @@
     return pack
 
 
+def conv_compose_pack(w0, b0, w1, b1):
+    lib = library()
+    arrays = [np.ascontiguousarray(a, dtype=np.float32)
+              for a in (w0, b0, w1, b1)]
+    assert arrays[0].shape == arrays[2].shape == (80, 80, 3)
+    assert arrays[1].shape == arrays[3].shape == (80,)
+    pack = np.zeros(lib.emph_conv_compose_pack_size(), dtype=np.float32)
+    check(lib.emph_conv_compose_pack(
+        *[a.ctypes.data for a in arrays], pack.ctypes.data),
+        'emph_conv_compose_pack')
+    return pack
+
+
 def conv_split_pack(weight):
     lib = library()
     weight = np.ascontiguousarray(weight, dtype=np.float32)
diff --git a/include/emphases_hip.h b/include/emphases_hip.h
--- a/include/emphases_hip.h
+++ b/include/emphases_hip.h
@@ -7,7 +7,7 @@
 extern "C" {
 #endif
 
-#define EMPH_ABI_VERSION 38
+#define EMPH_ABI_VERSION 39
 
 enum {
     EMPH_SEG_AUDIO_OFF = 0,
@@ -200,6 +200,16 @@
                       const float* packs, const float* biases, int32_t layers,
                       int32_t relu_mask, const int32_t* spans, int32_t n_spans,
                       const int32_t* slot_map, void* stream);
+
+int64_t emph_conv_compose_pack_size(void);
+int emph_conv_compose_pack(const float* w0, const float* b0, const float* w1,
+                           const float* b1, float* host_pack);
+int emph_conv1d_stack_composed(const float* x, int64_t ldx, float* y,
+                               int64_t ldy, const float* compose,
+                               const float* packs, const float* biases,
+                               int32_t layers, int32_t relu_mask,
+                               const int32_t* spans, int32_t n_spans,
+                               const int32_t* slot_map, void* stream);
 
 int64_t emph_conv_split_pack_size(void);
 int emph_conv_split_pack(const float* host_weight, void* host_pack);
@@ -437,6 +447,7 @@
     const float* decoder_biases;
     const float* out_weight;
     const float* out_bias;
+    const float* compose;
 } emph_conv_model;
 
 typedef struct emph_word_sum_tables {
```

Measured after the change: 463,700 utterances/s (median of 6 runs). +6.4%, better.
